# greysun/GraphEmbeddings

Hardware: AMD Instinct MI355X
Metric: scored triples/sec/GPU (d=200) (higher is better)
Workload: dtype f32

## Files before the change

### graphembeddings_amd/csrc/ge_launch.h

```cpp
#pragma once
#include <assert.h>
#include <hip/hip_runtime.h>
#include <stddef.h>
#include <stdint.h>

#include "ge_step_id.h"
#include "ge_sweep_route.h"
#include "ge_trans.h"

namespace ge {

struct TileGeom;
struct ShardOut;

int complex_max_dim();
int complex_score_launch(const float* table, int64_t N, int32_t d, const int32_t* triples, int64_t B, float max_norm,
                         int apply_sigmoid, float* out, hipStream_t st, int spectral = 0, float label = 0.f, float l2 = 0.f,
                         const float* table_sumsq = nullptr, int64_t ld = 0);
int complex_hinge_loss_launch(const float* table, int64_t N, int32_t d, const int32_t* pos, const int32_t* neg, int64_t B,
                              float margin, float max_norm, float* loss, float* sig_out, hipStream_t st, int spectral = 0);
int complex_hinge_grad_launch(const float* rows, int64_t N, int32_t d, const int32_t* pos, const int32_t* neg, int64_t B,
                              float margin, float lr, float max_norm, float* loss, int32_t* grad_idx, float* grad_val,
                              hipStream_t st, hipEvent_t ev_start = nullptr, hipEvent_t ev_stop = nullptr,
                              const int32_t* slot_item = nullptr, float* table_rw = nullptr, int spectral = 0,
                              const int32_t* order = nullptr);
int complex_logloss_grad_launch(const float* rows, int64_t N, int32_t d, const int32_t* triples, const float* labels,
                                int64_t M, float lr, float max_norm, float l2, const float* table_sumsq, float* loss,
                                int32_t* grad_idx, float* grad_val, hipStream_t st, const int32_t* negs = nullptr,
                                int64_t B = 0, float row_scale = 1.f, float neg_lr_eff = 0.f, hipEvent_t ev_start = nullptr,
                                hipEvent_t ev_stop = nullptr);
int shard_hinge_grad_launch(float* shard, int32_t d, const float* staged, const int32_t* pos_src, const int32_t* neg_src,
                            const int32_t* slot_item, int32_t R, int64_t B, float margin, float lr, float max_norm,
                            float* loss, int32_t* grad_idx, float* grad_val, float* gsum, int spectral, hipStream_t st,
                            hipEvent_t ev_start, hipEvent_t ev_stop, const int32_t* order, const float* const* peers,
                            int n_peers);
int table_sumsq_launch(const float* table, int64_t n, float* out, hipStream_t st);
int table_scale_launch(float* table, int64_t n, float factor, hipStream_t st);

int hole_score_launch(const float* table, int64_t N, int32_t d, const int32_t* triples, int64_t B, float max_norm,
                      int apply_sigmoid, float* out, hipStream_t st);
int hole_hinge_loss_launch(const float* table, int64_t N, int32_t d, const int32_t* pos, const int32_t* neg, int64_t B,
                           float margin, float max_norm, float* loss, float* sig_out, hipStream_t st);
int hole_hinge_grad_launch(const float* rows, int64_t N, int32_t d, const int32_t* pos, const int32_t* neg, int64_t B,
                           float margin, float lr, float max_norm, float* loss, int32_t* grad_idx, float* grad_val,
                           hipStream_t st, hipEvent_t ev_start = nullptr, hipEvent_t ev_stop = nullptr);

int hole_spectral_launch(float* table, int64_t N, int32_t d, int inverse, hipStream_t st);

int scatter_add_rows_launch(float* table, int64_t N, int32_t d, const int32_t* idx, const float* val, int64_t R,
                            hipStream_t st, hipEvent_t ev_start = nullptr, hipEvent_t ev_stop = nullptr);
int gather_rows_launch(const float* table, int64_t N, int32_t d, const int32_t* idx, int64_t R, float* out, hipStream_t st);
int corrupt_batch_launch(const int32_t* pos, int64_t B, const TypeSampler& ts, uint64_t step, int32_t* neg, hipStream_t st);
struct SamplerArgs {
  const int32_t* triples; int64_t T; const int64_t* bh_key; const int32_t* bh_ent; const int64_t* bt_key;
  const int32_t* bt_ent; int64_t n_known; const uint32_t* tail_threshold; int32_t n_rel, n_ent;
};
int bernoulli_corrupt_launch(const int32_t* pos, int64_t B, const SamplerArgs& s, int32_t ent_lo, uint64_t seed,
                             uint64_t step, int32_t* neg, hipStream_t st);
int select_rows_launch(const int32_t* valid, int64_t V, int64_t B, uint64_t seed, uint64_t counter, int32_t* out,
                       hipStream_t st);
int mean_pocket_launch(const float* loss, int64_t B, float* mean_out, float* best, int32_t* flag, hipStream_t st);
int copy_if_launch(const float* src, float* dst, int64_t n, const int32_t* flag, hipStream_t st);

int complex_score_1vK_launch(const float* table, int64_t N, int32_t d, const int32_t* hr, int64_t B, const int32_t* cand,
                             int64_t K, float max_norm, int apply_sigmoid, int cand_is_head, float* out, hipStream_t st);

struct SweepArgs {
  const float* table; int64_t N; int32_t d; const int32_t* hr; int64_t B; const int32_t* true_id; const int32_t* cand;
  int64_t K; float max_norm; int cand_is_head; const int32_t* known_off; const uint16_t* known_rc; int32_t* raw_cnt;
  int32_t* skip_cnt; float* true_loss; float* scores_out; int spec, scores_only, sweep_flags;
};
inline int table_mod16(const SweepArgs& a) { return (int)(reinterpret_cast<uintptr_t>(a.table) % 16); }
struct TopkOut { int32_t k; int32_t* out_id; float* out_loss; void* workspace; size_t workspace_bytes; };
struct SetArgs {
  const int32_t* row_set; const uint32_t* mask; int32_t n_sets;
  int64_t mw;
};

int complex_rank_1vK_launch(const SweepArgs& a, const void* planes_ws, hipStream_t st);

int pipe_sweep_launch(int cw, const SweepArgs& a, hipStream_t st);

int rank_planes_launch(const float* table, int64_t N, int32_t d, const int32_t* cand, int64_t K, float max_norm, int spec,
                       void* planes_ws, hipStream_t st);
int f16_sweep_launch(const SweepArgs& a, const void* planes_ws, hipStream_t st);
int topk_f16_launch(const SweepArgs& a, const TopkOut& t, const void* planes_ws, hipStream_t st);

int64_t candidate_mask_words(int64_t K);
int mask_from_classes_launch(const int32_t* cand_class, int64_t K, const uint32_t* allow, int32_t n_sets, int32_t n_class,
                             uint32_t* mask, hipStream_t st);
int mask_from_cells_launch(const int32_t* cells, int64_t M, int32_t n_sets, int64_t K, uint32_t* mask, hipStream_t st);
int masked_rank_launch(const SweepArgs& a, const SetArgs& sets, const void* planes_ws, hipStream_t st);
int masked_topk_launch(const SweepArgs& a, const TopkOut& t, const SetArgs& sets, const void* planes_ws, hipStream_t st);

int neighbor_max_k();
int neighbor_max_dim();
int64_t neighbor_planes_bytes(int64_t K, int32_t d);
int neighbor_planes_launch(const float* table, int64_t N, int32_t d, const int32_t* cand, int64_t K, void* planes_ws,
                           hipStream_t st);
size_t neighbor_ws_bytes(int64_t B, int64_t K, int32_t k);
int neighbor_dists_launch(const float* table, int64_t N, int32_t d, const int32_t* queries, int64_t B,
                          const int32_t* cand, int64_t K, int metric, const void* planes_ws, float* out, hipStream_t st);
int neighbor_topk_launch(const float* table, int64_t N, int32_t d, const int32_t* queries, int64_t B,
                         const int32_t* cand, int64_t K, int32_t k, int metric, int exclude_self, const void* planes_ws,
                         int32_t* out_id, float* out_dist, void* workspace, size_t workspace_bytes, hipStream_t st);

int known_cells_launch(int pass, const int64_t* key, const int64_t* ent, int64_t M, const int64_t* fixed, const int64_t* rel,
                       int64_t B, const int64_t* pos_of, int64_t n_rows, int64_t n_cand, int32_t* tile_cnt, int32_t* off,
                       uint16_t* rc, hipStream_t st);

size_t sort_scratch_bytes(int64_t n, int64_t n_sub, int64_t P);
unsigned long long* sort_scratch_keys(void* scratch);
int sort_tiles_launch(void* scratch, int64_t n, int64_t n_sub, int64_t P, int64_t n_rows, hipStream_t st,
                      const unsigned* limit, const unsigned long long** sorted);
int items_launch(const unsigned long long* sorted, int64_t n, const TileGeom& G, int direct, int32_t* out, const ShardOut* so,
                 hipStream_t st);
int relation_order_launch(const int32_t* triples, int64_t T, int64_t first_row, int64_t B, int64_t s0, int64_t n, int64_t N,
                          int32_t* out, int64_t stride, int64_t off_order, void* scratch, hipStream_t st);
size_t prep_big_scratch_bytes(int64_t B, int64_t negs, int64_t n);
int prepare_big_launch(const StepSeq& q, int64_t s0, int64_t n, const TypeSampler& ts, int direct, int32_t* out,
                       void* scratch, hipStream_t st, int negs);

int apply_items_launch(float* table, int d, const TileGeom& G, const int32_t* step_rec, const int32_t* gidx,
                       const float* gval, int split, float* out2, hipStream_t st, hipEvent_t ev_start, hipEvent_t ev_stop,
                       int det);
template <class T>
inline T* ws_at(void* base, size_t off) { return reinterpret_cast<T*>(reinterpret_cast<uintptr_t>(base) + off); }
struct HingeWs { int32_t* gidx; float* gval; size_t bytes; };
HingeWs hinge_ws(void* base, int64_t B, int32_t d);
struct LoglossWs { float* sumsq; int32_t* gidx; float* gval; size_t bytes; };
LoglossWs logloss_ws(void* base, int64_t M, int32_t d);
struct StepHyper {
  float lr0, decay_steps, decay_rate, max_norm;
  float lr_at(uint64_t gs) const { return decay_steps > 0.f ? lr0 / (1.0f + decay_rate * ((float)gs / decay_steps)) : lr0; }
};
size_t train_ws_bytes(int64_t B, int32_t d);
int train_steps_run(float* table, int32_t d, const StepSeq& q, int64_t n_steps, const TypeSampler& ts, float margin,
                    const StepHyper& hp, int model, float* loss, int keep_all_losses, int32_t* neg_ws, void* workspace,
                    size_t workspace_bytes, void** ev_pairs, int ev_kernel, void* pipe_handle, hipStream_t st);
size_t train_logloss_ws_bytes(int64_t B, int32_t negs, int32_t d);
int train_logloss_run(float* table, int32_t d, const StepSeq& q, int64_t n_steps, const TypeSampler& ts, int32_t negs,
                      float l2, const StepHyper& hp, float* loss, int keep_all_losses, int32_t* neg_ws, void* workspace,
                      size_t workspace_bytes, void* pipe_handle, hipStream_t st);
size_t train_prepare_bytes(int64_t B, int64_t n_steps);
int train_prepare_run(const StepSeq& q, int64_t n_steps, const TypeSampler& ts, int direct, int32_t* out, hipStream_t st);
void train_prepared_layout(int64_t B, int64_t* out);
int train_adagrad_run(float* table, float* accum, int32_t d, const StepSeq& q, int64_t n_steps, const TypeSampler& ts,
                      float margin, const StepHyper& hp, int model, float* loss, int keep_all_losses, int32_t* neg_ws,
                      void* workspace, size_t workspace_bytes, void* pipe_handle, hipStream_t st);
int pipeline_create(void** out);
int pipeline_reset(void* h);
int pipeline_destroy(void* h);

int adagrad_items_launch(float* table, float* accum, int d, const TileGeom& G, const int32_t* step_rec, const int32_t* gidx,
                         float* gval, float lr, hipStream_t st);
int adagrad_rows_launch(float* table, float* accum, int64_t N, int32_t d, const int32_t* idx, const float* val,
                        const int32_t* perm, int64_t R, float lr, hipStream_t st);

size_t shard_plan_scratch_bytes(int64_t B, int64_t S);
int shard_plan_launch(const int32_t* pos, const int32_t* neg, int64_t S, int64_t B, int64_t N, int32_t G, int32_t rank,
                      int32_t* records, int32_t* pos_src, int32_t* neg_src, int32_t* req_row, int32_t* counts,
                      void* scratch, int peer, hipStream_t st);
int shard_grad_launch(float* shard, int32_t d, const float* staged, const int32_t* pos_src, const int32_t* neg_src,
                      const int32_t* record, int32_t R, int64_t B, float margin, float lr, float max_norm, int spectral,
                      float* loss, int32_t* gidx, float* gval, float* gsum, const float* const* peers, int n_peers,
                      hipStream_t st, hipEvent_t e0, hipEvent_t e1);
int shard_apply_launch(float* shard, int32_t d, const int32_t* record, int64_t B, const int32_t* gidx, const float* gval,
                       int32_t R, float* gsum, hipStream_t st, hipEvent_t e0, hipEvent_t e1);
int64_t shard_owner_record_words(int64_t cap);
size_t shard_owner_scratch_bytes(int64_t cap, int64_t S);
int shard_owner_plan_launch(const int32_t* req_all, const int64_t* req_start, int64_t S, int64_t cap, int32_t rows_local,
                            int32_t* records, void* scratch, hipStream_t st);
int shard_owner_apply_launch(float* shard, int32_t d, const int32_t* record, int64_t cap, const float* recv, hipStream_t st);

int transx_max_dim();
size_t transx_ws_bytes(int64_t E, int64_t R, int32_t d, int64_t B);
int transx_score_launch(const TransModel& m, const int32_t* tri, int64_t B, float* out, hipStream_t st);
int transx_hinge_step_run(int model, int l1, float* ent, int64_t E, float* rel, int64_t R, float* normal,
                          float* ent_transfer, float* rel_transfer, int32_t d, const int32_t* pos, const int32_t* neg,
                          int64_t B, float margin, float lr, float* loss, void* workspace, size_t workspace_bytes,
                          hipStream_t st);
int transx_draw_launch(const SamplerArgs& s, int64_t B, uint64_t seed, uint64_t step, int32_t* pos, int32_t* neg,
                       hipStream_t st);
template <class Step>
int draw_then_step(const SamplerArgs& sa, int64_t B, uint64_t seed, uint64_t first_step, int64_t n_steps, int32_t* pos,
                   int32_t* neg, hipStream_t st, Step step) {
  for (int64_t s = 0; s < n_steps; ++s) {
    int rc = transx_draw_launch(sa, B, seed, first_step + (uint64_t)s, pos, neg, st);
    if (rc || (rc = step(s))) return rc;
  }
  return 0;
}
int transx_train_steps_run(int model, int l1, float* ent, int64_t E, float* rel, int64_t R, float* normal,
                           float* ent_transfer, float* rel_transfer, int32_t d, const SamplerArgs& sa, uint64_t seed,
                           uint64_t first_step, int64_t n_steps, int64_t B, float margin, float lr, float* losses,
                           void* workspace, size_t workspace_bytes, hipStream_t st);

int transr_max_dim();
size_t transr_ws_bytes(int64_t E, int64_t R, int32_t dE, int32_t dR, int64_t B);
int transr_score_launch(const TransModel& m, const int32_t* tri, int64_t B, float* out, hipStream_t st);
int transr_adam_step_run(int l1, float* ent, int64_t E, float* rel, float* rel_matrix, int64_t R, int32_t dE,
                         int32_t dR, float* m, float* v, const int32_t* pos, const int32_t* neg, int64_t B,
                         float margin, float lr, float b1, float b2, float eps, int64_t t, float* loss,
                         void* workspace, size_t workspace_bytes, hipStream_t st);
int transr_train_steps_run(int l1, float* ent, int64_t E, float* rel, float* rel_matrix, int64_t R, int32_t dE,
                           int32_t dR, float* m, float* v, const SamplerArgs& sa, uint64_t seed, uint64_t first_step,
                           int64_t n_steps, int64_t B, float margin, float lr, float b1, float b2, float eps,
                           int64_t first_t, float* losses, void* workspace, size_t workspace_bytes, hipStream_t st);

struct RankOut {
  const int32_t* known_off; const uint16_t* known_rc; int32_t* n_before; int32_t* n_known_before; float* true_dist;
  float* scores_out;
};

size_t trans_rank_ws_bytes(const TransModel& m, int64_t B);
int trans_rank_launch(const TransModel& m, const int32_t* tri, int64_t B, int cand_is_head, const RankOut& o,
                      void* workspace, size_t workspace_bytes, hipStream_t st);
int transx_topk_max_k();
size_t trans_topk_ws_bytes(const TransModel& m, int64_t B, int32_t k);
int trans_topk_launch(const TransModel& m, const int32_t* queries, int64_t B, int cand_is_head,
                      const int32_t* known_off, const uint16_t* known_rc, int32_t k, int32_t* out_id, float* out_dist,
                      void* workspace, size_t workspace_bytes, hipStream_t st);
int trans_rank_masked_launch(const TransModel& m, const int32_t* tri, int64_t B, int cand_is_head, const RankOut& o,
                             const SetArgs& sets, void* workspace, size_t workspace_bytes, hipStream_t st);
int trans_topk_masked_launch(const TransModel& m, const int32_t* queries, int64_t B, int cand_is_head,
                             const int32_t* known_off, const uint16_t* known_rc, int32_t k, int32_t* out_id,
                             float* out_dist, const SetArgs& sets, void* workspace, size_t workspace_bytes,
                             hipStream_t st);

size_t trans_relrank_ws_bytes(const TransModel& m, int64_t B);
int trans_relrank_launch(const TransModel& m, const int32_t* tri, int64_t B, const RankOut& o, void* workspace,
                         size_t workspace_bytes, hipStream_t st);

size_t threshold_fit_ws_bytes(int64_t M, int32_t n_seg);
int threshold_fit_launch(const float* score, const int32_t* seg, const uint8_t* label, int64_t M, int32_t n_seg,
                         float* thr_lo, float* thr_hi, int32_t* best_correct, int32_t* n_pos, int32_t* n_neg,
                         void* workspace, hipStream_t st);
int threshold_classify_launch(const float* score, const int32_t* seg, const uint8_t* label, int64_t M, int32_t n_seg,
                              const float* thr, uint8_t* pred, int32_t* confusion, hipStream_t st);

}
```

### graphembeddings_amd/csrc/ge_prep_big.hip

```cpp
#include "ge_prep.h"
#include "ge_launch.h"
#include <algorithm>

namespace ge {

__global__ __launch_bounds__(kPrepThreads) void prep_big_keys_kernel(
    const int32_t* __restrict__ triples, int64_t T, int64_t first_row, int64_t B, int64_t s0,
    const int32_t* __restrict__ id_to_type, int64_t N, const int64_t* __restrict__ type_offsets,
    int32_t n_types, const int32_t* __restrict__ type_ids, uint64_t seed, uint64_t global_step0,
    int32_t padded_size, int32_t mode, int direct, int negs, int32_t* __restrict__ prep,
    unsigned long long* __restrict__ keys_out) {
  const PrepLayout L = prep_layout(B, negs);
  const int tid = threadIdx.x, sub = blockIdx.y;
  const int64_t s = s0 + blockIdx.x;
  int32_t* rec = prep + (int64_t)blockIdx.x * L.stride;
  int32_t* slot_item = rec + L.off_slot;
  const int64_t i0 = (int64_t)sub * kSub;
  const int S = (int)((L.units - i0) < kSub ? (L.units - i0) : kSub);
  StepSource src{triples + 3 * step_row(first_row, T, B, s), B, id_to_type, N, type_offsets, n_types, type_ids, seed,
                 global_step0 + (uint64_t)s, padded_size, mode, negs};
  const bool batch_heads = (mode == GE_CORRUPT_BATCH_COIN) ? batch_coin_heads(seed, src.step) : false;
  unsigned long long* out = keys_out + ((int64_t)blockIdx.x * L.n_sub + sub) * L.P;
  if (direct)
    for (int i = tid; i < 6 * S; i += kPrepThreads) slot_item[6 * i0 + i] = -1;
  for (int il = tid; il < (int)L.S; il += kPrepThreads) {
    unsigned long long k[4] = {kInvalidKey, kInvalidKey, kInvalidKey, kInvalidKey};
    if (il < S) unit_keys(src, i0 + il, batch_heads, rec, k);
#pragma unroll
    for (int X = 0; X < 4; ++X)
      if (X < L.epu) out[L.epu * il + X] = k[X];
  }
}

__device__ __forceinline__ bool pass_is_identity(const unsigned* limit, int shift) {
  return limit && ((unsigned long long)(*limit) >> (shift - 32)) == 0ull;
}

__global__ __launch_bounds__(kPrepThreads) void prep_big_hist_kernel(
    const unsigned long long* __restrict__ src, int P, int n_sub, int shift, int bits, unsigned* __restrict__ hist,
    const unsigned* __restrict__ limit) {
  __shared__ unsigned cnt[kMaxRadix];
  if (pass_is_identity(limit, shift)) return;
  const int tid = threadIdx.x, tile = blockIdx.y;
  const int radix = 1 << bits;
  const unsigned dmask = (unsigned)radix - 1u;
  if (tid < radix) cnt[tid] = 0;
  __syncthreads();
  const unsigned long long* k = src + ((int64_t)blockIdx.x * n_sub + tile) * P;
  for (int i = tid; i < P; i += kPrepThreads) atomicAdd(&cnt[(unsigned)(k[i] >> shift) & dmask], 1u);
  __syncthreads();
  if (tid < radix) hist[((int64_t)blockIdx.x * radix + tid) * n_sub + tile] = cnt[tid];
}

__global__ __launch_bounds__(kPrepThreads) void prep_big_scatter_kernel(
    const unsigned long long* __restrict__ src, unsigned long long* __restrict__ dst,
    const unsigned* __restrict__ hist, int P, int n_sub, int shift, int bits, const unsigned* __restrict__ limit) {
  __shared__ unsigned whist[kMaxRadix * kPrepWaves];
  __shared__ unsigned gbase[kMaxRadix];
  __shared__ unsigned dstart[kMaxRadix];
  __shared__ unsigned wsum[4], wsum2[4];
  extern __shared__ __attribute__((aligned(16))) unsigned long long lkeys[];
  const int tid = threadIdx.x, lane = tid & (kWave - 1), wave = tid >> 6, tile = blockIdx.y;
  if (pass_is_identity(limit, shift)) {
    const int64_t o = ((int64_t)blockIdx.x * n_sub + tile) * P;
    for (int i = tid; i < P; i += kPrepThreads) dst[o + i] = src[o + i];
    return;
  }
  const int radix = 1 << bits, R = P / kPrepThreads, seg = kWave * R;
  const unsigned dmask = (unsigned)radix - 1u;
  const unsigned* h = hist + (int64_t)blockIdx.x * radix * n_sub;
  unsigned tot = 0, before = 0, mine = 0;
  if (tid < radix)
    for (int q = 0; q < n_sub; ++q) { const unsigned v = h[tid * n_sub + q]; if (q < tile) before += v; if (q == tile) mine = v; tot += v; }
  int incl = 0, incl2 = 0;
  if (tid < kMaxRadix) {
    incl = wave_incl_add((int)tot, lane);
    incl2 = wave_incl_add((int)mine, lane);
    if (lane == kWave - 1) { wsum[wave] = (unsigned)incl; wsum2[wave] = (unsigned)incl2; }
  }
  for (int i = tid; i < radix * kPrepWaves; i += kPrepThreads) whist[i] = 0;
  __syncthreads();
  if (tid < radix) {
    unsigned run = (unsigned)incl - tot, run2 = (unsigned)incl2 - mine;
    for (int w = 0; w < wave; ++w) { run += wsum[w]; run2 += wsum2[w]; }
    gbase[tid] = run + before;
    dstart[tid] = run2;
  }
  const unsigned long long* kin = src + ((int64_t)blockIdx.x * n_sub + tile) * P;
  unsigned long long k[16];
  unsigned off[16];
#pragma unroll
  for (int r = 0; r < 16; ++r)
    if (r < R) k[r] = kin[wave * seg + r * kWave + lane];
#pragma unroll
  for (int r = 0; r < 16; ++r) {
    if (r < R) {
      const unsigned dg = (unsigned)(k[r] >> shift) & dmask;
      unsigned long long peers = ~0ull;
      for (int b = 0; b < bits; ++b) {
        const bool bit = (dg >> b) & 1u;
        const unsigned long long bal = __ballot(bit);
        peers &= bit ? bal : ~bal;
      }
      const unsigned rank = (unsigned)__popcll(peers & ((1ull << lane) - 1ull));
      const unsigned cnt = (unsigned)__popcll(peers);
      unsigned* hp = whist + dg * kPrepWaves + wave;
      const unsigned base = *hp;
      __builtin_amdgcn_wave_barrier();
      if (rank == 0) *hp = base + cnt;
      __builtin_amdgcn_wave_barrier();
      off[r] = base + rank;
    }
  }
  __syncthreads();
  if (tid < radix) {
    unsigned run = 0;
    for (int w = 0; w < kPrepWaves; ++w) { const unsigned c = whist[tid * kPrepWaves + w]; whist[tid * kPrepWaves + w] = run; run += c; }
  }
  __syncthreads();
#pragma unroll
  for (int r = 0; r < 16; ++r) {
    if (r < R) {
      const unsigned dg = (unsigned)(k[r] >> shift) & dmask;
      lkeys[dstart[dg] + whist[dg * kPrepWaves + wave] + off[r]] = k[r];
    }
  }
  __syncthreads();
  unsigned long long* out = dst + (int64_t)blockIdx.x * n_sub * P;
  for (int i = tid; i < P; i += kPrepThreads) {
    const unsigned long long kk = lkeys[i];
    const unsigned dg = (unsigned)(kk >> shift) & dmask;
    out[gbase[dg] + ((unsigned)i - dstart[dg])] = kk;
  }
}

template <bool SHARD>
__global__ __launch_bounds__(kPrepThreads) void prep_big_items_kernel(
    const unsigned long long* __restrict__ sorted, TileGeom G, int direct, int32_t* __restrict__ prep, ShardOut so) {
  extern __shared__ __attribute__((aligned(16))) unsigned long long keys[];
  const int P = G.P, R = P / kPrepThreads, seg = kWave * R, n_sub = G.n_sub;
  int* wtot = reinterpret_cast<int*>(keys + P);
  const int tid = threadIdx.x, lane = tid & (kWave - 1), wave = tid >> 6, tile = blockIdx.y;
  const unsigned long long* g = sorted + (int64_t)blockIdx.x * n_sub * P;
  const int total = n_sub * P, base = tile * P;
  int32_t* rec = prep + (int64_t)blockIdx.x * G.stride;
  int32_t* slot_item = G.off_slot >= 0 ? rec + G.off_slot : nullptr;
  int32_t* subrec = rec + G.off_sub + tile * G.sub_stride;
  int32_t* items = subrec + G.off_items;
  int32_t* islots = subrec + G.off_islots;
  for (int i = tid; i < P; i += kPrepThreads) keys[i] = g[base + i];
  if (tid == 0) {
    int rs = -1;
    if (tile > 0) {
      const unsigned long long k0 = g[base], kp = g[base - 1];
      const uint32_t r0 = (uint32_t)(k0 >> 32);
      if (k0 != kInvalidKey && (uint32_t)(kp >> 32) == r0) {
        int lo = 0, hi = base - 1;
        while (lo < hi) { const int mid = (lo + hi) >> 1; if ((uint32_t)(g[mid] >> 32) < r0) lo = mid + 1; else hi = mid; }
        rs = lo;
      }
    }
    wtot[31] = rs;
    int before = 0;
    if (SHARD)
      for (int t = 0; t < tile; ++t) before += so.tile_heads[(int64_t)blockIdx.x * n_sub + t];
    wtot[30] = before;
  }
  __syncthreads();
  const int rs_in = wtot[31], u_before = wtot[30];
  auto key_at = [&](int i) -> unsigned long long {
    if (i >= 0 && i < P) return keys[i];
    const int gi = base + i;
    return (gi >= 0 && gi < total) ? g[gi] : kInvalidKey;
  };
  {
    int carry = -1;
    for (int r = 0; r < R; ++r) {
      const int i = wave * seg + r * kWave + lane;
      const unsigned long long kk = keys[i], kp = key_at(i - 1);
      const bool head = kk != kInvalidKey && (base + i == 0 || (uint32_t)(kp >> 32) != (uint32_t)(kk >> 32));
      const int m = max(wave_incl_max(head ? base + i : -1, lane), carry);
      carry = __shfl(m, kWave - 1, kWave);
    }
    if (lane == 0) wtot[wave] = carry;
  }
  __syncthreads();
  int prev_max = rs_in;
  for (int w = 0; w < wave; ++w) prev_max = max(prev_max, wtot[w]);
  __syncthreads();
  unsigned start_mask = 0, sole_mask = 0, rhead_mask = 0;
  int inc_loc[16], rs_loc[16];
  {
    int carry = 0, mcarry = prev_max;
#pragma unroll
    for (int r = 0; r < 16; ++r) {
      if (r < R) {
        const int i = wave * seg + r * kWave + lane;
        const unsigned long long kk = keys[i], kp = key_at(i - 1), kn = key_at(i + 1);
        const bool valid = kk != kInvalidKey;
        const uint32_t row = (uint32_t)(kk >> 32);
        const bool head = valid && (base + i == 0 || (uint32_t)(kp >> 32) != row);
        const bool sole = direct && head && !(kn != kInvalidKey && (uint32_t)(kn >> 32) == row) &&
                          !(SHARD && so.peer && row < (uint32_t)so.R);
        const bool rhead = SHARD && head && row >= (uint32_t)so.R;
        const int rs = max(wave_incl_max(head ? base + i : -1, lane), mcarry);
        mcarry = __shfl(rs, kWave - 1, kWave);
        rs_loc[r] = rs;
        const bool start = valid && ((base + i - rs) % kItemCap) == 0 && !sole;
        if (start) start_mask |= 1u << r;
        if (sole) sole_mask |= 1u << r;
        if (rhead) rhead_mask |= 1u << r;
        const int incl = wave_incl_add((start ? 1 : 0) | (rhead ? 1 << 16 : 0), lane) + carry;
        inc_loc[r] = incl;
        carry = __shfl(incl, kWave - 1, kWave);
      }
    }
    if (lane == 0) wtot[wave] = carry;
  }
  __syncthreads();
  int prev = 0, all = 0;
  for (int w = 0; w < kPrepWaves; ++w) { if (w < wave) prev += wtot[w]; all += wtot[w]; }
  if (tid == 0) subrec[0] = all & 0xFFFF;
  const int prev_items = prev & 0xFFFF, u0 = u_before + (prev >> 16) - 1;
#pragma unroll
  for (int r = 0; r < 16; ++r) {
    if (r < R) {
      const int i = wave * seg + r * kWave + lane;
      const unsigned long long kk = keys[i];
      const bool valid = kk != kInvalidKey;
      uint32_t row = (uint32_t)(kk >> 32);
      const uint32_t slot = (uint32_t)kk;
      const bool sole = (sole_mask >> r) & 1u;
      int tag = kSlotDirect;
      if (SHARD && valid) {
        const bool remote = row >= (uint32_t)so.R;
        const int u = u0 + (inc_loc[r] >> 16);
        uint32_t src = row;
        if (remote) {
          if ((rhead_mask >> r) & 1u) so.req_row[(int64_t)blockIdx.x * total + u] = (int32_t)(row % (uint32_t)so.R);
          if (!so.peer) src = (uint32_t)so.R + (uint32_t)u;
          row = (uint32_t)so.R + (uint32_t)u;
          tag = -3 - u;
        }
        const uint32_t pair = slot / 6u, X = slot - pair * 6u;
        if (X < 3) so.pos_src[((int64_t)blockIdx.x * so.B + pair) * 3 + X] = (int32_t)src;
        else so.neg_src[(int64_t)blockIdx.x * so.B + pair] = (int32_t)((src << 1) | (X - 3u));
      }
      if (sole) slot_item[slot] = tag;
      const bool is_start = (start_mask >> r) & 1u;
      unsigned long long sm = __ballot(is_start);
      const int idx_me = prev_items + (inc_loc[r] & 0xFFFF) - 1;
      const int g16 = lane >> 4, j16 = lane & 15;
      while (sm) {
        int srcl = -1;
#pragma unroll
        for (int g = 0; g < 4; ++g) {
          const int bpos = sm ? __builtin_ctzll(sm) : -1;
          if (sm) sm &= sm - 1;
          if (g == g16) srcl = bpos;
        }
        const int sl = srcl < 0 ? 0 : srcl;
        const int i_s = wave * seg + r * kWave + sl;
        const int idx_s = __shfl(idx_me, sl, kWave);
        const int row_s = __shfl((int)row, sl, kWave);
        const int rs_s = __shfl(rs_loc[r], sl, kWave);
        const unsigned long long k0 = key_at(i_s);
        const uint32_t krow = (uint32_t)(k0 >> 32);
        const unsigned long long kj = key_at(i_s + j16);
        const bool same = srcl >= 0 && kj != kInvalidKey && (uint32_t)(kj >> 32) == krow;
        const unsigned m16 = (unsigned)((__ballot(same) >> (16 * g16)) & 0xFFFFull);
        const int cnt = m16 == 0xFFFFu ? kItemCap : __builtin_ctz(~m16);
        if (srcl >= 0) {
          islots[idx_s * kItemCap + j16] = j16 < cnt ? (int32_t)(uint32_t)kj : -1;
          if (j16 == 0) {
            bool more = false;
            if (cnt == kItemCap) { const unsigned long long ke = key_at(i_s + kItemCap); more = ke != kInvalidKey && (uint32_t)(ke >> 32) == krow; }
            const bool multi = (base + i_s != rs_s) || more;
            items[2 * idx_s] = row_s;
            items[2 * idx_s + 1] = cnt | (multi ? (1 << 30) : 0);
          }
        }
      }
    }
  }
}

constexpr int kOrderP = 16384;
__global__ __launch_bounds__(kPrepThreads) void order_keys_kernel(
    const int32_t* __restrict__ triples, int64_t T, int64_t first_row, int64_t B, int64_t s0, int64_t N, int n_o,
    unsigned long long* __restrict__ keys_out, unsigned* __restrict__ limit) {
  const int64_t s = blockIdx.x;
  unsigned rmax = 0;
  const int32_t* pos = T > 0 ? triples + 3 * step_row(first_row, T, B, s0 + s) : triples + s * 3 * B;
  unsigned long long* out = keys_out + (s * n_o + blockIdx.y) * kOrderP;
  for (int i = threadIdx.x; i < kOrderP; i += kPrepThreads) {
    const int64_t j = (int64_t)blockIdx.y * kOrderP + i;
    unsigned long long k = kInvalidKey;
    if (j < B) {
      int32_t r = pos[3 * j + 2];
      if (r < 0 || r >= N) r = (int32_t)N;
      k = ((unsigned long long)(uint32_t)r << 32) | (uint32_t)j;
      rmax = max(rmax, (unsigned)r);
    }
    out[i] = k;
  }
#pragma unroll
  for (int m = 32; m >= 1; m >>= 1) rmax = max(rmax, (unsigned)__shfl_xor((int)rmax, m, kWave));
  if ((threadIdx.x & (kWave - 1)) == 0) atomicMax(limit, rmax);
}

__global__ __launch_bounds__(kPrepThreads) void order_write_kernel(
    const unsigned long long* __restrict__ sorted, int n_o, int64_t B, int64_t stride, int64_t off_order,
    int32_t* __restrict__ prep) {
  const unsigned long long* g = sorted + (int64_t)blockIdx.x * n_o * kOrderP;
  int32_t* order = prep + (int64_t)blockIdx.x * stride + off_order;
  for (int64_t i = (int64_t)blockIdx.y * kPrepThreads + threadIdx.x; i < B; i += (int64_t)gridDim.y * kPrepThreads)
    order[i] = (int32_t)(uint32_t)g[i];
}

size_t sort_scratch_bytes(int64_t n, int64_t n_sub, int64_t P) {
  const size_t keys = align_up(sizeof(unsigned long long) * (size_t)n * (size_t)n_sub * (size_t)P, 256);
  const size_t hist = align_up(sizeof(unsigned) * (size_t)n * kMaxRadix * (size_t)n_sub, 256);
  return 2 * keys + hist + 256;
}
static unsigned* sort_scratch_limit(void* scratch, int64_t n, int64_t n_sub, int64_t P) {
  return reinterpret_cast<unsigned*>(reinterpret_cast<char*>(scratch) + sort_scratch_bytes(n, n_sub, P) - 256);
}
unsigned long long* sort_scratch_keys(void* scratch) { return reinterpret_cast<unsigned long long*>(scratch); }

int sort_tiles_launch(void* scratch, int64_t n, int64_t n_sub, int64_t P, int64_t n_rows, hipStream_t st,
                      const unsigned* limit, const unsigned long long** sorted) {
  const SortBits sb = sort_bits_for(n_rows);
  const size_t keys_bytes = align_up(sizeof(unsigned long long) * (size_t)n * (size_t)n_sub * (size_t)P, 256);
  unsigned long long* ka = reinterpret_cast<unsigned long long*>(scratch);
  unsigned long long* kb = reinterpret_cast<unsigned long long*>(reinterpret_cast<char*>(scratch) + keys_bytes);
  unsigned* hist = reinterpret_cast<unsigned*>(reinterpret_cast<char*>(scratch) + 2 * keys_bytes);
  const dim3 grid((unsigned)n, (unsigned)n_sub), block(kPrepThreads);
  const size_t lds = sizeof(unsigned long long) * (size_t)P;
  const hipError_t e = hipFuncSetAttribute(reinterpret_cast<const void*>(prep_big_scatter_kernel),
                                           hipFuncAttributeMaxDynamicSharedMemorySize, 140 * 1024);
  if (e != hipSuccess) return (int)e;
  for (int pass = 0; pass < sb.n_pass; ++pass) {
    const int shift = 32 + pass * sb.bits;
    hipLaunchKernelGGL(prep_big_hist_kernel, grid, block, 0, st, ka, (int)P, (int)n_sub, shift, sb.bits, hist, limit);
    hipLaunchKernelGGL(prep_big_scatter_kernel, grid, block, lds, st, ka, kb, hist, (int)P, (int)n_sub, shift, sb.bits, limit);
    unsigned long long* t = ka; ka = kb; kb = t;
  }
  *sorted = ka;
  return launch_status();
}

int items_launch(const unsigned long long* sorted, int64_t n, const TileGeom& G, int direct, int32_t* out, const ShardOut* so,
                 hipStream_t st) {
  const size_t lds = sizeof(unsigned long long) * (size_t)G.P + sizeof(int) * 32;
  const dim3 grid((unsigned)n, (unsigned)G.n_sub), block(kPrepThreads);
  if (so) {
    hipError_t e = hipFuncSetAttribute(reinterpret_cast<const void*>(prep_big_items_kernel<true>),
                                       hipFuncAttributeMaxDynamicSharedMemorySize, 160 * 1024);
    if (e != hipSuccess) return (int)e;
    hipLaunchKernelGGL(prep_big_items_kernel<true>, grid, block, lds, st, sorted, G, direct, out, *so);
  } else {
    hipError_t e = hipFuncSetAttribute(reinterpret_cast<const void*>(prep_big_items_kernel<false>),
                                       hipFuncAttributeMaxDynamicSharedMemorySize, 160 * 1024);
    if (e != hipSuccess) return (int)e;
    hipLaunchKernelGGL(prep_big_items_kernel<false>, grid, block, lds, st, sorted, G, direct, out, ShardOut{});
  }
  return launch_status();
}

int relation_order_launch(const int32_t* triples, int64_t T, int64_t first_row, int64_t B, int64_t s0, int64_t n, int64_t N,
                          int32_t* out, int64_t stride, int64_t off_order, void* scratch, hipStream_t st) {
  const int n_o = (int)((B + kOrderP - 1) / kOrderP);
  unsigned* limit = sort_scratch_limit(scratch, n, n_o, kOrderP);
  if (hipMemsetAsync(limit, 0, sizeof(unsigned), st) != hipSuccess) return launch_status();
  hipLaunchKernelGGL(order_keys_kernel, dim3((unsigned)n, (unsigned)n_o), dim3(kPrepThreads), 0, st, triples, T, first_row, B,
                     s0, N, n_o, sort_scratch_keys(scratch), limit);
  const unsigned long long* sorted;
  const int rc = sort_tiles_launch(scratch, n, n_o, kOrderP, N + 1, st, limit, &sorted);
  if (rc) return rc;
  const int gy = (int)std::min<int64_t>((B + kPrepThreads - 1) / kPrepThreads, 64);
  hipLaunchKernelGGL(order_write_kernel, dim3((unsigned)n, (unsigned)gy), dim3(kPrepThreads), 0, st, sorted, n_o, B, stride,
                     off_order, out);
  return launch_status();
}

size_t prep_big_scratch_bytes(int64_t B, int64_t negs, int64_t n) {
  const PrepLayout L = prep_layout(B, negs);
  return L.n_sub <= 1 ? 0 : sort_scratch_bytes(n, L.n_sub, L.P);
}

int prepare_big_launch(const StepSeq& q, int64_t s0, int64_t n, const TypeSampler& ts, int direct, int32_t* out,
                       void* scratch, hipStream_t st, int negs) {
  const PrepLayout L = prep_layout(q.B, negs);
  const dim3 grid((unsigned)n, (unsigned)L.n_sub), block(kPrepThreads);
  hipLaunchKernelGGL(prep_big_keys_kernel, grid, block, 0, st, q.triples, q.T, q.first_row, q.B, s0, ts.id_to_type, ts.N,
                     ts.type_offsets, ts.n_types, ts.type_ids, ts.seed, q.global_step0, ts.padded_size, ts.mode, direct, negs,
                     out, sort_scratch_keys(scratch));
  const unsigned long long* sorted;
  int rc = sort_tiles_launch(scratch, n, L.n_sub, L.P, ts.N, st, nullptr, &sorted);
  if (rc) return rc;
  rc = items_launch(sorted, n, geom_of(L), direct, out, nullptr, st);
  if (rc || L.off_order < 0) return rc;
  return relation_order_launch(q.triples, q.T, q.first_row, q.B, s0, n, ts.N, out, L.stride, L.off_order, scratch, st);
}

}
```

### graphembeddings_amd/csrc/ge_shard.hip

```cpp
#include "ge_prep.h"
#include "ge_launch.h"

namespace ge {

__global__ __launch_bounds__(kPrepThreads) void shard_keys_kernel(
    const int32_t* __restrict__ pos, const int32_t* __restrict__ neg, int64_t B, int64_t N, int32_t G, int32_t rank,
    int32_t R, PrepLayout L, int32_t* __restrict__ prep, int32_t* __restrict__ pos_src, int32_t* __restrict__ neg_src,
    unsigned long long* __restrict__ keys_out) {
  const int tid = threadIdx.x, sub = blockIdx.y;
  const int64_t s = blockIdx.x;
  int32_t* slot_item = prep + s * L.stride + L.off_slot;
  const int64_t i0 = (int64_t)sub * kSub;
  const int S = (int)((B - i0) < kSub ? (B - i0) : kSub);
  unsigned long long* out = keys_out + (s * L.n_sub + sub) * L.P;
  for (int i = tid; i < 6 * S; i += kPrepThreads) slot_item[6 * i0 + i] = -1;
  auto vrow = [&](int32_t id) -> unsigned long long {
    const int32_t o = id % G, l = id / G;
    return (unsigned long long)(uint32_t)(o == rank ? l : R * (1 + o) + l);
  };
  for (int il = tid; il < (int)L.S; il += kPrepThreads) {
    unsigned long long k[4] = {kInvalidKey, kInvalidKey, kInvalidKey, kInvalidKey};
    if (il < S) {
      const int64_t i = i0 + il;
      const int32_t* p = pos + (s * B + i) * 3;
      const int32_t* n = neg + (s * B + i) * 3;
      const int32_t p0 = p[0], p1 = p[1], p2 = p[2], n0 = n[0], n1 = n[1], n2 = n[2];
      bool bad = p0 < 0 || p1 < 0 || p2 < 0 || p0 >= N || p1 >= N || p2 >= N || n0 < 0 || n1 < 0 || n0 >= N || n1 >= N;
      bad = bad || n2 != p2 || (n0 != p0 && n1 != p1);
      pos_src[(s * B + i) * 3] = -1; pos_src[(s * B + i) * 3 + 1] = -1; pos_src[(s * B + i) * 3 + 2] = -1;
      neg_src[s * B + i] = -1;
      if (!bad) {
        k[0] = (vrow(p0) << 32) | (uint32_t)(6 * i);
        k[1] = (vrow(p1) << 32) | (uint32_t)(6 * i + 1);
        k[2] = (vrow(p2) << 32) | (uint32_t)(6 * i + 2);
        if (n0 != p0) k[3] = (vrow(n0) << 32) | (uint32_t)(6 * i + 3);
        else if (n1 != p1) k[3] = (vrow(n1) << 32) | (uint32_t)(6 * i + 4);
      }
    }
#pragma unroll
    for (int X = 0; X < 4; ++X) out[4 * il + X] = k[X];
  }
}

__global__ __launch_bounds__(kPrepThreads) void shard_heads_kernel(
    const unsigned long long* __restrict__ sorted, int P, int n_sub, int32_t R, int32_t G, int32_t rank,
    int32_t* __restrict__ tile_heads, int32_t* __restrict__ counts) {
  __shared__ int own[64 + 1];
  const int tid = threadIdx.x, tile = blockIdx.y;
  const unsigned long long* g = sorted + (int64_t)blockIdx.x * n_sub * P;
  const int base = tile * P;
  if (tid <= 64) own[tid] = 0;
  __syncthreads();
  for (int i = tid; i < P; i += kPrepThreads) {
    const unsigned long long kk = g[base + i];
    if (kk == kInvalidKey) continue;
    const uint32_t row = (uint32_t)(kk >> 32);
    const bool head = (base + i == 0) || (uint32_t)(g[base + i - 1] >> 32) != row;
    if (!head) continue;
    if (row < (uint32_t)R) { atomicAdd(&own[rank], 1); continue; }
    atomicAdd(&own[row / (uint32_t)R - 1], 1);
    atomicAdd(&own[64], 1);
  }
  __syncthreads();
  if (tid < G && own[tid]) atomicAdd(&counts[(int64_t)blockIdx.x * G + tid], own[tid]);
  if (tid == 0) tile_heads[(int64_t)blockIdx.x * n_sub + tile] = own[64];
}

__global__ __launch_bounds__(kPrepThreads) void owner_keys_kernel(
    const int32_t* __restrict__ req_all, const int64_t* __restrict__ req_start, int P, int n_sub, int32_t rows_local,
    unsigned long long* __restrict__ keys_out) {
  const int64_t s = blockIdx.x;
  const int64_t b = req_start[s], n = req_start[s + 1] - b;
  unsigned long long* out = keys_out + (s * n_sub + blockIdx.y) * P;
  for (int i = threadIdx.x; i < P; i += kPrepThreads) {
    const int64_t j = (int64_t)blockIdx.y * P + i;
    unsigned long long k = kInvalidKey;
    if (j < n) {
      const int32_t row = req_all[b + j];
      if (row >= 0 && row < rows_local) k = ((unsigned long long)(uint32_t)row << 32) | (uint32_t)j;
    }
    out[i] = k;
  }
}

size_t shard_plan_scratch_bytes(int64_t B, int64_t S) {
  const PrepLayout L = prep_layout(B);
  return sort_scratch_bytes(S, L.n_sub, L.P) + align_up(sizeof(int32_t) * (size_t)S * (size_t)L.n_sub, 256);
}

int shard_plan_launch(const int32_t* pos, const int32_t* neg, int64_t S, int64_t B, int64_t N, int32_t G, int32_t rank,
                      int32_t* records, int32_t* pos_src, int32_t* neg_src, int32_t* req_row, int32_t* counts,
                      void* scratch, int peer, hipStream_t st) {
  const PrepLayout L = prep_layout(B);
  const int32_t R = (int32_t)((N + G - 1) / G);
  const dim3 grid((unsigned)S, (unsigned)L.n_sub), block(kPrepThreads);
  int32_t* tile_heads = reinterpret_cast<int32_t*>(reinterpret_cast<char*>(scratch) + sort_scratch_bytes(S, L.n_sub, L.P));
  hipError_t e = hipMemsetAsync(counts, 0, sizeof(int32_t) * (size_t)S * (size_t)G, st);
  if (e != hipSuccess) return (int)e;
  hipLaunchKernelGGL(shard_keys_kernel, grid, block, 0, st, pos, neg, B, N, G, rank, R, L, records, pos_src, neg_src,
                     sort_scratch_keys(scratch));
  const unsigned long long* sorted;
  int rc = sort_tiles_launch(scratch, S, L.n_sub, L.P, (int64_t)R * (G + 1), st, nullptr, &sorted);
  if (rc) return rc;
  hipLaunchKernelGGL(shard_heads_kernel, grid, block, 0, st, sorted, (int)L.P, (int)L.n_sub, R, G, rank, tile_heads, counts);
  const ShardOut so{R, B, pos_src, neg_src, req_row, tile_heads, peer ? 1 : 0};
  rc = items_launch(sorted, S, geom_of(L), 1, records, &so, st);
  if (rc || L.off_order < 0) return rc;
  return relation_order_launch(pos, 0, 0, B, 0, S, N, records, L.stride, L.off_order, scratch, st);
}

int shard_grad_launch(float* shard, int32_t d, const float* staged, const int32_t* pos_src, const int32_t* neg_src,
                      const int32_t* record, int32_t R, int64_t B, float margin, float lr, float max_norm, int spectral,
                      float* loss, int32_t* gidx, float* gval, float* gsum, const float* const* peers, int n_peers,
                      hipStream_t st, hipEvent_t e0, hipEvent_t e1) {
  const PrepLayout L = prep_layout(B);
  return shard_hinge_grad_launch(shard, d, staged, pos_src, neg_src, record + L.off_slot, R, B, margin, lr, max_norm, loss,
                                 gidx, gval, gsum, spectral, st, e0, e1, L.off_order >= 0 ? record + L.off_order : nullptr,
                                 peers, n_peers);
}

int shard_apply_launch(float* shard, int32_t d, const int32_t* record, int64_t B, const int32_t* gidx, const float* gval,
                       int32_t R, float* gsum, hipStream_t st, hipEvent_t e0, hipEvent_t e1) {
  return apply_items_launch(shard, d, geom_of(prep_layout(B)), record, gidx, gval, R, gsum, st, e0, e1, 0);
}

constexpr int kOwnerP = 16384;
static inline int owner_tiles(int64_t cap) { return (int)((cap + kOwnerP - 1) / kOwnerP); }
int64_t shard_owner_record_words(int64_t cap) { return cap <= 0 ? 0 : geom_plain(kOwnerP, owner_tiles(cap)).stride; }
size_t shard_owner_scratch_bytes(int64_t cap, int64_t S) { return cap <= 0 ? 0 : sort_scratch_bytes(S, owner_tiles(cap), kOwnerP); }

int shard_owner_plan_launch(const int32_t* req_all, const int64_t* req_start, int64_t S, int64_t cap, int32_t rows_local,
                            int32_t* records, void* scratch, hipStream_t st) {
  if (cap <= 0 || S <= 0) return 0;
  const int n_sub = owner_tiles(cap);
  const dim3 grid((unsigned)S, (unsigned)n_sub), block(kPrepThreads);
  hipLaunchKernelGGL(owner_keys_kernel, grid, block, 0, st, req_all, req_start, kOwnerP, n_sub, rows_local,
                     sort_scratch_keys(scratch));
  const unsigned long long* sorted;
  const int rc = sort_tiles_launch(scratch, S, n_sub, kOwnerP, rows_local, st, nullptr, &sorted);
  if (rc) return rc;
  return items_launch(sorted, S, geom_plain(kOwnerP, n_sub), 0, records, nullptr, st);
}

int shard_owner_apply_launch(float* shard, int32_t d, const int32_t* record, int64_t cap, const float* recv, hipStream_t st) {
  if (cap <= 0) return 0;
  return apply_items_launch(shard, d, geom_plain(kOwnerP, owner_tiles(cap)), record, nullptr, recv, 0x7FFFFFFF, nullptr, st,
                            nullptr, nullptr, 0);
}

}
```

Baseline: 593.9 million.

## Restructure prep radix sort into fixed-span blocks with fused key counting

Reworks the per-step radix sort used in batch preparation. Tiles of up to P keys per block become fixed 4096-key spans of 256-thread blocks processed in 1024-key rounds with static shared memory. The key-generation kernel now also builds the first-pass histogram, so one count kernel is skipped. The items kernel is split into a counting launch and a writing launch over 1024-key spans. The aim is more blocks, higher occupancy and no large dynamic LDS, at the cost of extra launches, more histogram traffic and more complex carry logic across spans.

```diff
diff --git a/graphembeddings_amd/csrc/ge_launch.h b/graphembeddings_amd/csrc/ge_launch.h
--- a/graphembeddings_amd/csrc/ge_launch.h
+++ b/graphembeddings_amd/csrc/ge_launch.h
@@ -112,9 +112,9 @@
 size_t sort_scratch_bytes(int64_t n, int64_t n_sub, int64_t P);
 unsigned long long* sort_scratch_keys(void* scratch);
 int sort_tiles_launch(void* scratch, int64_t n, int64_t n_sub, int64_t P, int64_t n_rows, hipStream_t st,
-                      const unsigned* limit, const unsigned long long** sorted);
+                      const unsigned long long** sorted);
 int items_launch(const unsigned long long* sorted, int64_t n, const TileGeom& G, int direct, int32_t* out, const ShardOut* so,
-                 hipStream_t st);
+                 void* scratch, hipStream_t st);
 int relation_order_launch(const int32_t* triples, int64_t T, int64_t first_row, int64_t B, int64_t s0, int64_t n, int64_t N,
                           int32_t* out, int64_t stride, int64_t off_order, void* scratch, hipStream_t st);
 size_t prep_big_scratch_bytes(int64_t B, int64_t negs, int64_t n);
diff --git a/graphembeddings_amd/csrc/ge_prep_big.hip b/graphembeddings_amd/csrc/ge_prep_big.hip
--- a/graphembeddings_amd/csrc/ge_prep_big.hip
+++ b/graphembeddings_amd/csrc/ge_prep_big.hip
@@ -4,97 +4,132 @@
 
 namespace ge {
 
-__global__ __launch_bounds__(kPrepThreads) void prep_big_keys_kernel(
+constexpr int kBigThreads = 256;
+constexpr int kBigWaves = kBigThreads / kWave;
+constexpr int kSortRound = 1024;
+constexpr int kSortR = kSortRound / kBigThreads;
+constexpr int kSortSpan = 4096;
+constexpr int kItemSpan = 1024;
+constexpr int kItemR = kItemSpan / kBigThreads;
+constexpr int kKeyUnits = 1024;
+static_assert(kMaxRadix <= kBigThreads, "one digit per thread in the scans");
+static_assert(kSortSpan % kSortRound == 0 && kSortRound % kBigThreads == 0 && kItemSpan % kBigThreads == 0, "geometry");
+
+static inline int64_t sort_spans(int64_t total) { return (total + kSortSpan - 1) / kSortSpan; }
+
+__device__ __forceinline__ void count_write(const unsigned* lcnt, unsigned* __restrict__ cnt, int n_span, int radix) {
+  if ((int)threadIdx.x < radix) cnt[((int64_t)blockIdx.x * n_span + blockIdx.y) * radix + threadIdx.x] = lcnt[threadIdx.x];
+}
+
+__global__ __launch_bounds__(kBigThreads) void prep_big_keys_kernel(
     const int32_t* __restrict__ triples, int64_t T, int64_t first_row, int64_t B, int64_t s0,
     const int32_t* __restrict__ id_to_type, int64_t N, const int64_t* __restrict__ type_offsets,
     int32_t n_types, const int32_t* __restrict__ type_ids, uint64_t seed, uint64_t global_step0,
     int32_t padded_size, int32_t mode, int direct, int negs, int32_t* __restrict__ prep,
-    unsigned long long* __restrict__ keys_out) {
+    unsigned long long* __restrict__ keys_out, unsigned* __restrict__ cnt, int bits) {
+  __shared__ unsigned lcnt[kMaxRadix];
   const PrepLayout L = prep_layout(B, negs);
-  const int tid = threadIdx.x, sub = blockIdx.y;
+  const int tid = threadIdx.x;
   const int64_t s = s0 + blockIdx.x;
   int32_t* rec = prep + (int64_t)blockIdx.x * L.stride;
   int32_t* slot_item = rec + L.off_slot;
-  const int64_t i0 = (int64_t)sub * kSub;
-  const int S = (int)((L.units - i0) < kSub ? (L.units - i0) : kSub);
+  const int pu0 = blockIdx.y * kKeyUnits, pu_end = (int)(L.n_sub * L.S), S = (int)L.S, units = (int)L.units;
   StepSource src{triples + 3 * step_row(first_row, T, B, s), B, id_to_type, N, type_offsets, n_types, type_ids, seed,
                  global_step0 + (uint64_t)s, padded_size, mode, negs};
   const bool batch_heads = (mode == GE_CORRUPT_BATCH_COIN) ? batch_coin_heads(seed, src.step) : false;
-  unsigned long long* out = keys_out + ((int64_t)blockIdx.x * L.n_sub + sub) * L.P;
+  unsigned long long* out = keys_out + (int64_t)blockIdx.x * L.n_sub * L.P;
+  const unsigned dmask = (1u << bits) - 1u;
+  if (cnt) {
+    lcnt[tid] = 0;
+    __syncthreads();
+  }
   if (direct)
-    for (int i = tid; i < 6 * S; i += kPrepThreads) slot_item[6 * i0 + i] = -1;
-  for (int il = tid; il < (int)L.S; il += kPrepThreads) {
+    for (int i = tid; i < 6 * kKeyUnits; i += kBigThreads) {
+      const int pu = pu0 + i / 6, tile = pu / S, j = tile * (int)kSub + (pu - tile * S);
+      if (pu < pu_end && j < units) slot_item[6 * (int64_t)j + i % 6] = -1;
+    }
+  for (int u = tid; u < kKeyUnits; u += kBigThreads) {
+    const int pu = pu0 + u;
+    if (pu >= pu_end) break;
+    const int tile = pu / S, j = tile * (int)kSub + (pu - tile * S);
     unsigned long long k[4] = {kInvalidKey, kInvalidKey, kInvalidKey, kInvalidKey};
-    if (il < S) unit_keys(src, i0 + il, batch_heads, rec, k);
+    if (j < units) unit_keys(src, j, batch_heads, rec, k);
 #pragma unroll
     for (int X = 0; X < 4; ++X)
-      if (X < L.epu) out[L.epu * il + X] = k[X];
+      if (X < L.epu) {
+        out[L.epu * (int64_t)pu + X] = k[X];
+        if (cnt) atomicAdd(&lcnt[(unsigned)(k[X] >> 32) & dmask], 1u);
+      }
+  }
+  if (cnt) {
+    __syncthreads();
+    count_write(lcnt, cnt, (int)gridDim.y, 1 << bits);
   }
 }
 
 __device__ __forceinline__ bool pass_is_identity(const unsigned* limit, int shift) {
   return limit && ((unsigned long long)(*limit) >> (shift - 32)) == 0ull;
 }
-
-__global__ __launch_bounds__(kPrepThreads) void prep_big_hist_kernel(
-    const unsigned long long* __restrict__ src, int P, int n_sub, int shift, int bits, unsigned* __restrict__ hist,
+__device__ __forceinline__ const unsigned long long* sorted_of(const unsigned long long* ka, const unsigned long long* kb,
+                                                               const unsigned* limit, int n_pass, int bits) {
+  int m = 0;
+  for (int p = 0; p < n_pass; ++p) m += pass_is_identity(limit, 32 + p * bits) ? 0 : 1;
+  return (m & 1) ? kb : ka;
+}
+
+__global__ __launch_bounds__(kBigThreads) void sort_count_kernel(
+    const unsigned long long* __restrict__ src, int total, int shift, int bits, unsigned* __restrict__ cnt,
     const unsigned* __restrict__ limit) {
-  __shared__ unsigned cnt[kMaxRadix];
+  __shared__ unsigned lcnt[kMaxRadix];
   if (pass_is_identity(limit, shift)) return;
-  const int tid = threadIdx.x, tile = blockIdx.y;
+  const int tid = threadIdx.x;
+  const unsigned dmask = (1u << bits) - 1u;
+  lcnt[tid] = 0;
+  __syncthreads();
+  const int p0 = blockIdx.y * kSortSpan, p1 = min(p0 + kSortSpan, total);
+  const unsigned long long* k = src + (int64_t)blockIdx.x * total;
+  for (int i = p0 + tid; i < p1; i += kBigThreads) atomicAdd(&lcnt[(unsigned)(k[i] >> shift) & dmask], 1u);
+  __syncthreads();
+  count_write(lcnt, cnt, (int)gridDim.y, 1 << bits);
+}
+
+__global__ __launch_bounds__(kBigThreads) void sort_scatter_kernel(
+    const unsigned long long* __restrict__ src, unsigned long long* __restrict__ dst, const unsigned* __restrict__ cnt,
+    int total, int shift, int bits, const unsigned* __restrict__ limit) {
+  __shared__ __attribute__((aligned(16))) unsigned long long lkeys[kSortRound];
+  __shared__ unsigned whist[kBigWaves * kMaxRadix];
+  __shared__ unsigned gbase[kMaxRadix];
+  __shared__ unsigned dstart[kMaxRadix];
+  __shared__ unsigned wsum[kBigWaves], wsum2[kBigWaves];
+  if (pass_is_identity(limit, shift)) return;
+  const int tid = threadIdx.x, lane = tid & (kWave - 1), wave = tid >> 6, span = blockIdx.y, n_span = gridDim.y;
   const int radix = 1 << bits;
   const unsigned dmask = (unsigned)radix - 1u;
-  if (tid < radix) cnt[tid] = 0;
-  __syncthreads();
-  const unsigned long long* k = src + ((int64_t)blockIdx.x * n_sub + tile) * P;
-  for (int i = tid; i < P; i += kPrepThreads) atomicAdd(&cnt[(unsigned)(k[i] >> shift) & dmask], 1u);
-  __syncthreads();
-  if (tid < radix) hist[((int64_t)blockIdx.x * radix + tid) * n_sub + tile] = cnt[tid];
-}
-
-__global__ __launch_bounds__(kPrepThreads) void prep_big_scatter_kernel(
-    const unsigned long long* __restrict__ src, unsigned long long* __restrict__ dst,
-    const unsigned* __restrict__ hist, int P, int n_sub, int shift, int bits, const unsigned* __restrict__ limit) {
-  __shared__ unsigned whist[kMaxRadix * kPrepWaves];
-  __shared__ unsigned gbase[kMaxRadix];
-  __shared__ unsigned dstart[kMaxRadix];
-  __shared__ unsigned wsum[4], wsum2[4];
-  extern __shared__ __attribute__((aligned(16))) unsigned long long lkeys[];
-  const int tid = threadIdx.x, lane = tid & (kWave - 1), wave = tid >> 6, tile = blockIdx.y;
-  if (pass_is_identity(limit, shift)) {
-    const int64_t o = ((int64_t)blockIdx.x * n_sub + tile) * P;
-    for (int i = tid; i < P; i += kPrepThreads) dst[o + i] = src[o + i];
-    return;
-  }
-  const int radix = 1 << bits, R = P / kPrepThreads, seg = kWave * R;
-  const unsigned dmask = (unsigned)radix - 1u;
-  const unsigned* h = hist + (int64_t)blockIdx.x * radix * n_sub;
-  unsigned tot = 0, before = 0, mine = 0;
-  if (tid < radix)
-    for (int q = 0; q < n_sub; ++q) { const unsigned v = h[tid * n_sub + q]; if (q < tile) before += v; if (q == tile) mine = v; tot += v; }
-  int incl = 0, incl2 = 0;
-  if (tid < kMaxRadix) {
-    incl = wave_incl_add((int)tot, lane);
-    incl2 = wave_incl_add((int)mine, lane);
-    if (lane == kWave - 1) { wsum[wave] = (unsigned)incl; wsum2[wave] = (unsigned)incl2; }
-  }
-  for (int i = tid; i < radix * kPrepWaves; i += kPrepThreads) whist[i] = 0;
-  __syncthreads();
+  unsigned tot = 0, before = 0;
   if (tid < radix) {
-    unsigned run = (unsigned)incl - tot, run2 = (unsigned)incl2 - mine;
-    for (int w = 0; w < wave; ++w) { run += wsum[w]; run2 += wsum2[w]; }
-    gbase[tid] = run + before;
-    dstart[tid] = run2;
-  }
-  const unsigned long long* kin = src + ((int64_t)blockIdx.x * n_sub + tile) * P;
-  unsigned long long k[16];
-  unsigned off[16];
-#pragma unroll
-  for (int r = 0; r < 16; ++r)
-    if (r < R) k[r] = kin[wave * seg + r * kWave + lane];
-#pragma unroll
-  for (int r = 0; r < 16; ++r) {
-    if (r < R) {
+    const unsigned* h = cnt + (int64_t)blockIdx.x * n_span * radix + tid;
+#pragma unroll 4
+    for (int q = 0; q < n_span; ++q) { const unsigned v = h[(int64_t)q * radix]; if (q < span) before += v; tot += v; }
+  }
+  const int incl = wave_incl_add((int)tot, lane);
+  if (lane == kWave - 1) wsum[wave] = (unsigned)incl;
+  __syncthreads();
+  unsigned my_base = (unsigned)incl - tot + before;
+#pragma unroll
+  for (int w = 0; w < kBigWaves; ++w) my_base += w < wave ? wsum[w] : 0u;
+  gbase[tid] = my_base;
+  const int p0 = span * kSortSpan, rounds = min(kSortSpan, total - p0) / kSortRound;
+  const unsigned long long* kin = src + (int64_t)blockIdx.x * total + p0;
+  unsigned long long* out = dst + (int64_t)blockIdx.x * total;
+  for (int t = 0; t < rounds; ++t) {
+    for (int i = tid; i < kMaxRadix * kBigWaves; i += kBigThreads) whist[i] = 0;
+    __syncthreads();
+    unsigned long long k[kSortR];
+    unsigned off[kSortR];
+#pragma unroll
+    for (int r = 0; r < kSortR; ++r) k[r] = kin[t * kSortRound + wave * (kWave * kSortR) + r * kWave + lane];
+#pragma unroll
+    for (int r = 0; r < kSortR; ++r) {
       const unsigned dg = (unsigned)(k[r] >> shift) & dmask;
       unsigned long long peers = ~0ull;
       for (int b = 0; b < bits; ++b) {
@@ -103,55 +138,65 @@
         peers &= bit ? bal : ~bal;
       }
       const unsigned rank = (unsigned)__popcll(peers & ((1ull << lane) - 1ull));
-      const unsigned cnt = (unsigned)__popcll(peers);
-      unsigned* hp = whist + dg * kPrepWaves + wave;
+      const unsigned c = (unsigned)__popcll(peers);
+      unsigned* hp = whist + wave * kMaxRadix + dg;
       const unsigned base = *hp;
       __builtin_amdgcn_wave_barrier();
-      if (rank == 0) *hp = base + cnt;
+      if (rank == 0) *hp = base + c;
       __builtin_amdgcn_wave_barrier();
       off[r] = base + rank;
     }
-  }
-  __syncthreads();
-  if (tid < radix) {
-    unsigned run = 0;
-    for (int w = 0; w < kPrepWaves; ++w) { const unsigned c = whist[tid * kPrepWaves + w]; whist[tid * kPrepWaves + w] = run; run += c; }
-  }
-  __syncthreads();
-#pragma unroll
-  for (int r = 0; r < 16; ++r) {
-    if (r < R) {
+    __syncthreads();
+    unsigned mine = 0;
+    if (tid < radix)
+      for (int w = 0; w < kBigWaves; ++w) { const unsigned c = whist[w * kMaxRadix + tid]; whist[w * kMaxRadix + tid] = mine; mine += c; }
+    const int incl2 = wave_incl_add((int)mine, lane);
+    if (lane == kWave - 1) wsum2[wave] = (unsigned)incl2;
+    __syncthreads();
+    unsigned ds = (unsigned)incl2 - mine;
+#pragma unroll
+    for (int w = 0; w < kBigWaves; ++w) ds += w < wave ? wsum2[w] : 0u;
+    dstart[tid] = ds;
+    __syncthreads();
+#pragma unroll
+    for (int r = 0; r < kSortR; ++r) {
       const unsigned dg = (unsigned)(k[r] >> shift) & dmask;
-      lkeys[dstart[dg] + whist[dg * kPrepWaves + wave] + off[r]] = k[r];
-    }
-  }
-  __syncthreads();
-  unsigned long long* out = dst + (int64_t)blockIdx.x * n_sub * P;
-  for (int i = tid; i < P; i += kPrepThreads) {
-    const unsigned long long kk = lkeys[i];
-    const unsigned dg = (unsigned)(kk >> shift) & dmask;
-    out[gbase[dg] + ((unsigned)i - dstart[dg])] = kk;
-  }
-}
-
-template <bool SHARD>
-__global__ __launch_bounds__(kPrepThreads) void prep_big_items_kernel(
-    const unsigned long long* __restrict__ sorted, TileGeom G, int direct, int32_t* __restrict__ prep, ShardOut so) {
-  extern __shared__ __attribute__((aligned(16))) unsigned long long keys[];
-  const int P = G.P, R = P / kPrepThreads, seg = kWave * R, n_sub = G.n_sub;
-  int* wtot = reinterpret_cast<int*>(keys + P);
-  const int tid = threadIdx.x, lane = tid & (kWave - 1), wave = tid >> 6, tile = blockIdx.y;
+      lkeys[dstart[dg] + whist[wave * kMaxRadix + dg] + off[r]] = k[r];
+    }
+    __syncthreads();
+    for (int i = tid; i < kSortRound; i += kBigThreads) {
+      const unsigned long long kk = lkeys[i];
+      const unsigned dg = (unsigned)(kk >> shift) & dmask;
+      out[gbase[dg] + ((unsigned)i - dstart[dg])] = kk;
+    }
+    __syncthreads();
+    my_base += mine;
+    gbase[tid] = my_base;
+  }
+}
+
+template <bool SHARD, bool COUNT>
+__global__ __launch_bounds__(kBigThreads) void items_kernel(
+    const unsigned long long* __restrict__ sorted, TileGeom G, int direct, int32_t* __restrict__ prep, ShardOut so,
+    int32_t* __restrict__ span_cnt) {
+  __shared__ __attribute__((aligned(16))) unsigned long long keys[kItemSpan];
+  __shared__ int wtot[kBigWaves], carry_in[3];
+  constexpr int seg = kWave * kItemR;
+  const int P = G.P, n_sub = G.n_sub, spt = P / kItemSpan;
+  const int tid = threadIdx.x, lane = tid & (kWave - 1), wave = tid >> 6;
+  const int tile = blockIdx.y / spt, sp = blockIdx.y - tile * spt;
   const unsigned long long* g = sorted + (int64_t)blockIdx.x * n_sub * P;
-  const int total = n_sub * P, base = tile * P;
+  const int total = n_sub * P, base = blockIdx.y * kItemSpan;
+  int32_t* cnt_tile = span_cnt + ((int64_t)blockIdx.x * n_sub + tile) * spt;
   int32_t* rec = prep + (int64_t)blockIdx.x * G.stride;
   int32_t* slot_item = G.off_slot >= 0 ? rec + G.off_slot : nullptr;
   int32_t* subrec = rec + G.off_sub + tile * G.sub_stride;
   int32_t* items = subrec + G.off_items;
   int32_t* islots = subrec + G.off_islots;
-  for (int i = tid; i < P; i += kPrepThreads) keys[i] = g[base + i];
+  for (int i = tid; i < kItemSpan; i += kBigThreads) keys[i] = g[base + i];
   if (tid == 0) {
     int rs = -1;
-    if (tile > 0) {
+    if (base > 0) {
       const unsigned long long k0 = g[base], kp = g[base - 1];
       const uint32_t r0 = (uint32_t)(k0 >> 32);
       if (k0 != kInvalidKey && (uint32_t)(kp >> 32) == r0) {
@@ -160,22 +205,29 @@
         rs = lo;
       }
     }
-    wtot[31] = rs;
-    int before = 0;
-    if (SHARD)
-      for (int t = 0; t < tile; ++t) before += so.tile_heads[(int64_t)blockIdx.x * n_sub + t];
-    wtot[30] = before;
-  }
-  __syncthreads();
-  const int rs_in = wtot[31], u_before = wtot[30];
+    carry_in[0] = rs;
+    if (!COUNT) {
+      int prev = 0, all = 0;
+      for (int q = 0; q < spt; ++q) { const int c = cnt_tile[q]; if (q < sp) prev += c; all += c; }
+      int before = 0;
+      if (SHARD)
+        for (int t = 0; t < tile; ++t) before += so.tile_heads[(int64_t)blockIdx.x * n_sub + t];
+      carry_in[1] = prev;
+      carry_in[2] = before;
+      if (sp == 0) subrec[0] = all & 0xFFFF;
+    }
+  }
+  __syncthreads();
+  const int rs_in = carry_in[0];
   auto key_at = [&](int i) -> unsigned long long {
-    if (i >= 0 && i < P) return keys[i];
+    if (i >= 0 && i < kItemSpan) return keys[i];
     const int gi = base + i;
     return (gi >= 0 && gi < total) ? g[gi] : kInvalidKey;
   };
   {
     int carry = -1;
-    for (int r = 0; r < R; ++r) {
+#pragma unroll
+    for (int r = 0; r < kItemR; ++r) {
       const int i = wave * seg + r * kWave + lane;
       const unsigned long long kk = keys[i], kp = key_at(i - 1);
       const bool head = kk != kInvalidKey && (base + i == 0 || (uint32_t)(kp >> 32) != (uint32_t)(kk >> 32));
@@ -189,181 +241,189 @@
   for (int w = 0; w < wave; ++w) prev_max = max(prev_max, wtot[w]);
   __syncthreads();
   unsigned start_mask = 0, sole_mask = 0, rhead_mask = 0;
-  int inc_loc[16], rs_loc[16];
+  int inc_loc[kItemR], rs_loc[kItemR];
   {
     int carry = 0, mcarry = prev_max;
 #pragma unroll
-    for (int r = 0; r < 16; ++r) {
-      if (r < R) {
-        const int i = wave * seg + r * kWave + lane;
-        const unsigned long long kk = keys[i], kp = key_at(i - 1), kn = key_at(i + 1);
-        const bool valid = kk != kInvalidKey;
-        const uint32_t row = (uint32_t)(kk >> 32);
-        const bool head = valid && (base + i == 0 || (uint32_t)(kp >> 32) != row);
-        const bool sole = direct && head && !(kn != kInvalidKey && (uint32_t)(kn >> 32) == row) &&
-                          !(SHARD && so.peer && row < (uint32_t)so.R);
-        const bool rhead = SHARD && head && row >= (uint32_t)so.R;
-        const int rs = max(wave_incl_max(head ? base + i : -1, lane), mcarry);
-        mcarry = __shfl(rs, kWave - 1, kWave);
-        rs_loc[r] = rs;
-        const bool start = valid && ((base + i - rs) % kItemCap) == 0 && !sole;
-        if (start) start_mask |= 1u << r;
-        if (sole) sole_mask |= 1u << r;
-        if (rhead) rhead_mask |= 1u << r;
-        const int incl = wave_incl_add((start ? 1 : 0) | (rhead ? 1 << 16 : 0), lane) + carry;
-        inc_loc[r] = incl;
-        carry = __shfl(incl, kWave - 1, kWave);
-      }
+    for (int r = 0; r < kItemR; ++r) {
+      const int i = wave * seg + r * kWave + lane;
+      const unsigned long long kk = keys[i], kp = key_at(i - 1), kn = key_at(i + 1);
+      const bool valid = kk != kInvalidKey;
+      const uint32_t row = (uint32_t)(kk >> 32);
+      const bool head = valid && (base + i == 0 || (uint32_t)(kp >> 32) != row);
+      const bool sole = direct && head && !(kn != kInvalidKey && (uint32_t)(kn >> 32) == row) &&
+                        !(SHARD && so.peer && row < (uint32_t)so.R);
+      const bool rhead = SHARD && head && row >= (uint32_t)so.R;
+      const int rs = max(wave_incl_max(head ? base + i : -1, lane), mcarry);
+      mcarry = __shfl(rs, kWave - 1, kWave);
+      rs_loc[r] = rs;
+      const bool start = valid && ((base + i - rs) % kItemCap) == 0 && !sole;
+      if (start) start_mask |= 1u << r;
+      if (sole) sole_mask |= 1u << r;
+      if (rhead) rhead_mask |= 1u << r;
+      const int incl = wave_incl_add((start ? 1 : 0) | (rhead ? 1 << 16 : 0), lane) + carry;
+      inc_loc[r] = incl;
+      carry = __shfl(incl, kWave - 1, kWave);
     }
     if (lane == 0) wtot[wave] = carry;
   }
   __syncthreads();
-  int prev = 0, all = 0;
-  for (int w = 0; w < kPrepWaves; ++w) { if (w < wave) prev += wtot[w]; all += wtot[w]; }
-  if (tid == 0) subrec[0] = all & 0xFFFF;
-  const int prev_items = prev & 0xFFFF, u0 = u_before + (prev >> 16) - 1;
-#pragma unroll
-  for (int r = 0; r < 16; ++r) {
-    if (r < R) {
-      const int i = wave * seg + r * kWave + lane;
-      const unsigned long long kk = keys[i];
-      const bool valid = kk != kInvalidKey;
-      uint32_t row = (uint32_t)(kk >> 32);
-      const uint32_t slot = (uint32_t)kk;
-      const bool sole = (sole_mask >> r) & 1u;
-      int tag = kSlotDirect;
-      if (SHARD && valid) {
-        const bool remote = row >= (uint32_t)so.R;
-        const int u = u0 + (inc_loc[r] >> 16);
-        uint32_t src = row;
-        if (remote) {
-          if ((rhead_mask >> r) & 1u) so.req_row[(int64_t)blockIdx.x * total + u] = (int32_t)(row % (uint32_t)so.R);
-          if (!so.peer) src = (uint32_t)so.R + (uint32_t)u;
-          row = (uint32_t)so.R + (uint32_t)u;
-          tag = -3 - u;
+  if (COUNT) {
+    if (tid == 0) { int all = 0; for (int w = 0; w < kBigWaves; ++w) all += wtot[w]; cnt_tile[sp] = all; }
+    return;
+  }
+  int prev = carry_in[1];
+  for (int w = 0; w < wave; ++w) prev += wtot[w];
+  const int prev_items = prev & 0xFFFF, u0 = carry_in[2] + (prev >> 16) - 1;
+#pragma unroll
+  for (int r = 0; r < kItemR; ++r) {
+    const int i = wave * seg + r * kWave + lane;
+    const unsigned long long kk = keys[i];
+    const bool valid = kk != kInvalidKey;
+    uint32_t row = (uint32_t)(kk >> 32);
+    const uint32_t slot = (uint32_t)kk;
+    const bool sole = (sole_mask >> r) & 1u;
+    int tag = kSlotDirect;
+    if (SHARD && valid) {
+      const bool remote = row >= (uint32_t)so.R;
+      const int u = u0 + (inc_loc[r] >> 16);
+      uint32_t src = row;
+      if (remote) {
+        if ((rhead_mask >> r) & 1u) so.req_row[(int64_t)blockIdx.x * total + u] = (int32_t)(row % (uint32_t)so.R);
+        if (!so.peer) src = (uint32_t)so.R + (uint32_t)u;
+        row = (uint32_t)so.R + (uint32_t)u;
+        tag = -3 - u;
+      }
+      const uint32_t pair = slot / 6u, X = slot - pair * 6u;
+      if (X < 3) so.pos_src[((int64_t)blockIdx.x * so.B + pair) * 3 + X] = (int32_t)src;
+      else so.neg_src[(int64_t)blockIdx.x * so.B + pair] = (int32_t)((src << 1) | (X - 3u));
+    }
+    if (sole) slot_item[slot] = tag;
+    const bool is_start = (start_mask >> r) & 1u;
+    unsigned long long sm = __ballot(is_start);
+    const int idx_me = prev_items + (inc_loc[r] & 0xFFFF) - 1;
+    const int g16 = lane >> 4, j16 = lane & 15;
+    while (sm) {
+      int srcl = -1;
+#pragma unroll
+      for (int gq = 0; gq < 4; ++gq) {
+        const int bpos = sm ? __builtin_ctzll(sm) : -1;
+        if (sm) sm &= sm - 1;
+        if (gq == g16) srcl = bpos;
+      }
+      const int sl = srcl < 0 ? 0 : srcl;
+      const int i_s = wave * seg + r * kWave + sl;
+      const int idx_s = __shfl(idx_me, sl, kWave);
+      const int row_s = __shfl((int)row, sl, kWave);
+      const int rs_s = __shfl(rs_loc[r], sl, kWave);
+      const unsigned long long k0 = key_at(i_s);
+      const uint32_t krow = (uint32_t)(k0 >> 32);
+      const unsigned long long kj = key_at(i_s + j16);
+      const bool same = srcl >= 0 && kj != kInvalidKey && (uint32_t)(kj >> 32) == krow;
+      const unsigned m16 = (unsigned)((__ballot(same) >> (16 * g16)) & 0xFFFFull);
+      const int cnt = m16 == 0xFFFFu ? kItemCap : __builtin_ctz(~m16);
+      if (srcl >= 0) {
+        islots[idx_s * kItemCap + j16] = j16 < cnt ? (int32_t)(uint32_t)kj : -1;
+        if (j16 == 0) {
+          bool more = false;
+          if (cnt == kItemCap) { const unsigned long long ke = key_at(i_s + kItemCap); more = ke != kInvalidKey && (uint32_t)(ke >> 32) == krow; }
+          const bool multi = (base + i_s != rs_s) || more;
+          items[2 * idx_s] = row_s;
+          items[2 * idx_s + 1] = cnt | (multi ? (1 << 30) : 0);
         }
-        const uint32_t pair = slot / 6u, X = slot - pair * 6u;
-        if (X < 3) so.pos_src[((int64_t)blockIdx.x * so.B + pair) * 3 + X] = (int32_t)src;
-        else so.neg_src[(int64_t)blockIdx.x * so.B + pair] = (int32_t)((src << 1) | (X - 3u));
-      }
-      if (sole) slot_item[slot] = tag;
-      const bool is_start = (start_mask >> r) & 1u;
-      unsigned long long sm = __ballot(is_start);
-      const int idx_me = prev_items + (inc_loc[r] & 0xFFFF) - 1;
-      const int g16 = lane >> 4, j16 = lane & 15;
-      while (sm) {
-        int srcl = -1;
-#pragma unroll
-        for (int g = 0; g < 4; ++g) {
-          const int bpos = sm ? __builtin_ctzll(sm) : -1;
-          if (sm) sm &= sm - 1;
-          if (g == g16) srcl = bpos;
-        }
-        const int sl = srcl < 0 ? 0 : srcl;
-        const int i_s = wave * seg + r * kWave + sl;
-        const int idx_s = __shfl(idx_me, sl, kWave);
-        const int row_s = __shfl((int)row, sl, kWave);
-        const int rs_s = __shfl(rs_loc[r], sl, kWave);
-        const unsigned long long k0 = key_at(i_s);
-        const uint32_t krow = (uint32_t)(k0 >> 32);
-        const unsigned long long kj = key_at(i_s + j16);
-        const bool same = srcl >= 0 && kj != kInvalidKey && (uint32_t)(kj >> 32) == krow;
-        const unsigned m16 = (unsigned)((__ballot(same) >> (16 * g16)) & 0xFFFFull);
-        const int cnt = m16 == 0xFFFFu ? kItemCap : __builtin_ctz(~m16);
-        if (srcl >= 0) {
-          islots[idx_s * kItemCap + j16] = j16 < cnt ? (int32_t)(uint32_t)kj : -1;
-          if (j16 == 0) {
-            bool more = false;
-            if (cnt == kItemCap) { const unsigned long long ke = key_at(i_s + kItemCap); more = ke != kInvalidKey && (uint32_t)(ke >> 32) == krow; }
-            const bool multi = (base + i_s != rs_s) || more;
-            items[2 * idx_s] = row_s;
-            items[2 * idx_s + 1] = cnt | (multi ? (1 << 30) : 0);
-          }
-        }
       }
     }
   }
 }
 
 constexpr int kOrderP = 16384;
-__global__ __launch_bounds__(kPrepThreads) void order_keys_kernel(
-    const int32_t* __restrict__ triples, int64_t T, int64_t first_row, int64_t B, int64_t s0, int64_t N, int n_o,
-    unsigned long long* __restrict__ keys_out, unsigned* __restrict__ limit) {
+__global__ __launch_bounds__(kBigThreads) void order_keys_kernel(
+    const int32_t* __restrict__ triples, int64_t T, int64_t first_row, int64_t B, int64_t s0, int64_t N, int total,
+    unsigned long long* __restrict__ keys_out, unsigned* __restrict__ limit, unsigned* __restrict__ cnt, int bits) {
+  __shared__ unsigned lcnt[kMaxRadix];
   const int64_t s = blockIdx.x;
+  const unsigned dmask = (1u << bits) - 1u;
   unsigned rmax = 0;
   const int32_t* pos = T > 0 ? triples + 3 * step_row(first_row, T, B, s0 + s) : triples + s * 3 * B;
-  unsigned long long* out = keys_out + (s * n_o + blockIdx.y) * kOrderP;
-  for (int i = threadIdx.x; i < kOrderP; i += kPrepThreads) {
-    const int64_t j = (int64_t)blockIdx.y * kOrderP + i;
+  unsigned long long* out = keys_out + s * total;
+  lcnt[threadIdx.x] = 0;
+  __syncthreads();
+  const int p0 = blockIdx.y * kSortSpan, p1 = min(p0 + kSortSpan, total);
+  for (int j = p0 + threadIdx.x; j < p1; j += kBigThreads) {
     unsigned long long k = kInvalidKey;
     if (j < B) {
-      int32_t r = pos[3 * j + 2];
+      int32_t r = pos[3 * (int64_t)j + 2];
       if (r < 0 || r >= N) r = (int32_t)N;
       k = ((unsigned long long)(uint32_t)r << 32) | (uint32_t)j;
       rmax = max(rmax, (unsigned)r);
     }
-    out[i] = k;
+    out[j] = k;
+    atomicAdd(&lcnt[(unsigned)(k >> 32) & dmask], 1u);
   }
 #pragma unroll
   for (int m = 32; m >= 1; m >>= 1) rmax = max(rmax, (unsigned)__shfl_xor((int)rmax, m, kWave));
   if ((threadIdx.x & (kWave - 1)) == 0) atomicMax(limit, rmax);
-}
-
-__global__ __launch_bounds__(kPrepThreads) void order_write_kernel(
-    const unsigned long long* __restrict__ sorted, int n_o, int64_t B, int64_t stride, int64_t off_order,
-    int32_t* __restrict__ prep) {
-  const unsigned long long* g = sorted + (int64_t)blockIdx.x * n_o * kOrderP;
+  __syncthreads();
+  count_write(lcnt, cnt, (int)gridDim.y, 1 << bits);
+}
+
+__global__ __launch_bounds__(kBigThreads) void order_write_kernel(
+    const unsigned long long* __restrict__ ka, const unsigned long long* __restrict__ kb, const unsigned* __restrict__ limit,
+    int n_pass, int bits, int total, int64_t B, int64_t stride, int64_t off_order, int32_t* __restrict__ prep) {
+  const unsigned long long* g = sorted_of(ka, kb, limit, n_pass, bits) + (int64_t)blockIdx.x * total;
   int32_t* order = prep + (int64_t)blockIdx.x * stride + off_order;
-  for (int64_t i = (int64_t)blockIdx.y * kPrepThreads + threadIdx.x; i < B; i += (int64_t)gridDim.y * kPrepThreads)
+  for (int64_t i = (int64_t)blockIdx.y * kBigThreads + threadIdx.x; i < B; i += (int64_t)gridDim.y * kBigThreads)
     order[i] = (int32_t)(uint32_t)g[i];
 }
 
-size_t sort_scratch_bytes(int64_t n, int64_t n_sub, int64_t P) {
+struct SortScratch { unsigned long long *ka, *kb; unsigned *cnt, *limit; size_t bytes; };
+static SortScratch sort_scratch(void* scratch, int64_t n, int64_t n_sub, int64_t P) {
   const size_t keys = align_up(sizeof(unsigned long long) * (size_t)n * (size_t)n_sub * (size_t)P, 256);
-  const size_t hist = align_up(sizeof(unsigned) * (size_t)n * kMaxRadix * (size_t)n_sub, 256);
-  return 2 * keys + hist + 256;
-}
-static unsigned* sort_scratch_limit(void* scratch, int64_t n, int64_t n_sub, int64_t P) {
-  return reinterpret_cast<unsigned*>(reinterpret_cast<char*>(scratch) + sort_scratch_bytes(n, n_sub, P) - 256);
-}
+  const size_t cnt = align_up(sizeof(unsigned) * (size_t)n * kMaxRadix * (size_t)sort_spans(n_sub * P), 256);
+  return SortScratch{ws_at<unsigned long long>(scratch, 0), ws_at<unsigned long long>(scratch, keys),
+                     ws_at<unsigned>(scratch, 2 * keys), ws_at<unsigned>(scratch, 2 * keys + cnt), 2 * keys + cnt + 256};
+}
+size_t sort_scratch_bytes(int64_t n, int64_t n_sub, int64_t P) { return sort_scratch(nullptr, n, n_sub, P).bytes; }
 unsigned long long* sort_scratch_keys(void* scratch) { return reinterpret_cast<unsigned long long*>(scratch); }
 
-int sort_tiles_launch(void* scratch, int64_t n, int64_t n_sub, int64_t P, int64_t n_rows, hipStream_t st,
-                      const unsigned* limit, const unsigned long long** sorted) {
-  const SortBits sb = sort_bits_for(n_rows);
-  const size_t keys_bytes = align_up(sizeof(unsigned long long) * (size_t)n * (size_t)n_sub * (size_t)P, 256);
-  unsigned long long* ka = reinterpret_cast<unsigned long long*>(scratch);
-  unsigned long long* kb = reinterpret_cast<unsigned long long*>(reinterpret_cast<char*>(scratch) + keys_bytes);
-  unsigned* hist = reinterpret_cast<unsigned*>(reinterpret_cast<char*>(scratch) + 2 * keys_bytes);
-  const dim3 grid((unsigned)n, (unsigned)n_sub), block(kPrepThreads);
-  const size_t lds = sizeof(unsigned long long) * (size_t)P;
-  const hipError_t e = hipFuncSetAttribute(reinterpret_cast<const void*>(prep_big_scatter_kernel),
-                                           hipFuncAttributeMaxDynamicSharedMemorySize, 140 * 1024);
-  if (e != hipSuccess) return (int)e;
+static void sort_passes(const SortScratch& w, int64_t n, int64_t total, SortBits sb, bool counted0, const unsigned* limit,
+                        hipStream_t st) {
+  const dim3 grid((unsigned)n, (unsigned)sort_spans(total)), block(kBigThreads);
+  unsigned long long *ka = w.ka, *kb = w.kb;
   for (int pass = 0; pass < sb.n_pass; ++pass) {
     const int shift = 32 + pass * sb.bits;
-    hipLaunchKernelGGL(prep_big_hist_kernel, grid, block, 0, st, ka, (int)P, (int)n_sub, shift, sb.bits, hist, limit);
-    hipLaunchKernelGGL(prep_big_scatter_kernel, grid, block, lds, st, ka, kb, hist, (int)P, (int)n_sub, shift, sb.bits, limit);
-    unsigned long long* t = ka; ka = kb; kb = t;
-  }
-  *sorted = ka;
+    if (pass > 0 || !counted0)
+      hipLaunchKernelGGL(sort_count_kernel, grid, block, 0, st, ka, (int)total, shift, sb.bits, w.cnt, limit);
+    hipLaunchKernelGGL(sort_scatter_kernel, grid, block, 0, st, ka, kb, w.cnt, (int)total, shift, sb.bits, limit);
+#ifdef GE_EXP_PREP_REPEAT
+    for (int rep = 1; rep < GE_EXP_PREP_REPEAT; ++rep)
+      hipLaunchKernelGGL(sort_scatter_kernel, grid, block, 0, st, ka, kb, w.cnt, (int)total, shift, sb.bits, limit);
+#endif
+    std::swap(ka, kb);
+  }
+}
+
+int sort_tiles_launch(void* scratch, int64_t n, int64_t n_sub, int64_t P, int64_t n_rows, hipStream_t st,
+                      const unsigned long long** sorted) {
+  if (P % kSortRound) return GE_EINVAL;
+  const SortScratch w = sort_scratch(scratch, n, n_sub, P);
+  const SortBits sb = sort_bits_for(n_rows);
+  sort_passes(w, n, n_sub * P, sb, false, nullptr, st);
+  *sorted = (sb.n_pass & 1) ? w.kb : w.ka;
   return launch_status();
 }
 
 int items_launch(const unsigned long long* sorted, int64_t n, const TileGeom& G, int direct, int32_t* out, const ShardOut* so,
-                 hipStream_t st) {
-  const size_t lds = sizeof(unsigned long long) * (size_t)G.P + sizeof(int) * 32;
-  const dim3 grid((unsigned)n, (unsigned)G.n_sub), block(kPrepThreads);
+                 void* scratch, hipStream_t st) {
+  if (G.P % kItemSpan) return GE_EINVAL;
+  int32_t* span_cnt = reinterpret_cast<int32_t*>(sort_scratch(scratch, n, G.n_sub, G.P).cnt);
+  const dim3 grid((unsigned)n, (unsigned)(G.n_sub * (G.P / kItemSpan))), block(kBigThreads);
   if (so) {
-    hipError_t e = hipFuncSetAttribute(reinterpret_cast<const void*>(prep_big_items_kernel<true>),
-                                       hipFuncAttributeMaxDynamicSharedMemorySize, 160 * 1024);
-    if (e != hipSuccess) return (int)e;
-    hipLaunchKernelGGL(prep_big_items_kernel<true>, grid, block, lds, st, sorted, G, direct, out, *so);
+    hipLaunchKernelGGL((items_kernel<true, true>), grid, block, 0, st, sorted, G, direct, out, *so, span_cnt);
+    hipLaunchKernelGGL((items_kernel<true, false>), grid, block, 0, st, sorted, G, direct, out, *so, span_cnt);
   } else {
-    hipError_t e = hipFuncSetAttribute(reinterpret_cast<const void*>(prep_big_items_kernel<false>),
-                                       hipFuncAttributeMaxDynamicSharedMemorySize, 160 * 1024);
-    if (e != hipSuccess) return (int)e;
-    hipLaunchKernelGGL(prep_big_items_kernel<false>, grid, block, lds, st, sorted, G, direct, out, ShardOut{});
+    hipLaunchKernelGGL((items_kernel<false, true>), grid, block, 0, st, sorted, G, direct, out, ShardOut{}, span_cnt);
+    hipLaunchKernelGGL((items_kernel<false, false>), grid, block, 0, st, sorted, G, direct, out, ShardOut{}, span_cnt);
   }
   return launch_status();
 }
@@ -371,16 +431,16 @@
 int relation_order_launch(const int32_t* triples, int64_t T, int64_t first_row, int64_t B, int64_t s0, int64_t n, int64_t N,
                           int32_t* out, int64_t stride, int64_t off_order, void* scratch, hipStream_t st) {
   const int n_o = (int)((B + kOrderP - 1) / kOrderP);
-  unsigned* limit = sort_scratch_limit(scratch, n, n_o, kOrderP);
-  if (hipMemsetAsync(limit, 0, sizeof(unsigned), st) != hipSuccess) return launch_status();
-  hipLaunchKernelGGL(order_keys_kernel, dim3((unsigned)n, (unsigned)n_o), dim3(kPrepThreads), 0, st, triples, T, first_row, B,
-                     s0, N, n_o, sort_scratch_keys(scratch), limit);
-  const unsigned long long* sorted;
-  const int rc = sort_tiles_launch(scratch, n, n_o, kOrderP, N + 1, st, limit, &sorted);
-  if (rc) return rc;
-  const int gy = (int)std::min<int64_t>((B + kPrepThreads - 1) / kPrepThreads, 64);
-  hipLaunchKernelGGL(order_write_kernel, dim3((unsigned)n, (unsigned)gy), dim3(kPrepThreads), 0, st, sorted, n_o, B, stride,
-                     off_order, out);
+  const int64_t total = (int64_t)n_o * kOrderP;
+  const SortScratch w = sort_scratch(scratch, n, n_o, kOrderP);
+  const SortBits sb = sort_bits_for(N + 1);
+  if (hipMemsetAsync(w.limit, 0, sizeof(unsigned), st) != hipSuccess) return launch_status();
+  hipLaunchKernelGGL(order_keys_kernel, dim3((unsigned)n, (unsigned)sort_spans(total)), dim3(kBigThreads), 0, st, triples, T,
+                     first_row, B, s0, N, (int)total, w.ka, w.limit, w.cnt, sb.bits);
+  sort_passes(w, n, total, sb, true, w.limit, st);
+  const int gy = (int)std::min<int64_t>((B + kBigThreads - 1) / kBigThreads, 64);
+  hipLaunchKernelGGL(order_write_kernel, dim3((unsigned)n, (unsigned)gy), dim3(kBigThreads), 0, st, w.ka, w.kb, w.limit,
+                     sb.n_pass, sb.bits, (int)total, B, stride, off_order, out);
   return launch_status();
 }
 
@@ -392,14 +452,15 @@
 int prepare_big_launch(const StepSeq& q, int64_t s0, int64_t n, const TypeSampler& ts, int direct, int32_t* out,
                        void* scratch, hipStream_t st, int negs) {
   const PrepLayout L = prep_layout(q.B, negs);
-  const dim3 grid((unsigned)n, (unsigned)L.n_sub), block(kPrepThreads);
-  hipLaunchKernelGGL(prep_big_keys_kernel, grid, block, 0, st, q.triples, q.T, q.first_row, q.B, s0, ts.id_to_type, ts.N,
-                     ts.type_offsets, ts.n_types, ts.type_ids, ts.seed, q.global_step0, ts.padded_size, ts.mode, direct, negs,
-                     out, sort_scratch_keys(scratch));
-  const unsigned long long* sorted;
-  int rc = sort_tiles_launch(scratch, n, L.n_sub, L.P, ts.N, st, nullptr, &sorted);
-  if (rc) return rc;
-  rc = items_launch(sorted, n, geom_of(L), direct, out, nullptr, st);
+  const SortScratch w = sort_scratch(scratch, n, L.n_sub, L.P);
+  const SortBits sb = sort_bits_for(ts.N);
+  const int64_t total = L.n_sub * L.P, n_blk = (L.n_sub * L.S + kKeyUnits - 1) / kKeyUnits;
+  const bool counted0 = L.epu * kKeyUnits == kSortSpan;
+  hipLaunchKernelGGL(prep_big_keys_kernel, dim3((unsigned)n, (unsigned)n_blk), dim3(kBigThreads), 0, st, q.triples, q.T,
+                     q.first_row, q.B, s0, ts.id_to_type, ts.N, ts.type_offsets, ts.n_types, ts.type_ids, ts.seed,
+                     q.global_step0, ts.padded_size, ts.mode, direct, negs, out, w.ka, counted0 ? w.cnt : nullptr, sb.bits);
+  sort_passes(w, n, total, sb, counted0, nullptr, st);
+  int rc = items_launch((sb.n_pass & 1) ? w.kb : w.ka, n, geom_of(L), direct, out, nullptr, scratch, st);
   if (rc || L.off_order < 0) return rc;
   return relation_order_launch(q.triples, q.T, q.first_row, q.B, s0, n, ts.N, out, L.stride, L.off_order, scratch, st);
 }
diff --git a/graphembeddings_amd/csrc/ge_shard.hip b/graphembeddings_amd/csrc/ge_shard.hip
--- a/graphembeddings_amd/csrc/ge_shard.hip
+++ b/graphembeddings_amd/csrc/ge_shard.hip
@@ -100,11 +100,11 @@
   hipLaunchKernelGGL(shard_keys_kernel, grid, block, 0, st, pos, neg, B, N, G, rank, R, L, records, pos_src, neg_src,
                      sort_scratch_keys(scratch));
   const unsigned long long* sorted;
-  int rc = sort_tiles_launch(scratch, S, L.n_sub, L.P, (int64_t)R * (G + 1), st, nullptr, &sorted);
+  int rc = sort_tiles_launch(scratch, S, L.n_sub, L.P, (int64_t)R * (G + 1), st, &sorted);
   if (rc) return rc;
   hipLaunchKernelGGL(shard_heads_kernel, grid, block, 0, st, sorted, (int)L.P, (int)L.n_sub, R, G, rank, tile_heads, counts);
   const ShardOut so{R, B, pos_src, neg_src, req_row, tile_heads, peer ? 1 : 0};
-  rc = items_launch(sorted, S, geom_of(L), 1, records, &so, st);
+  rc = items_launch(sorted, S, geom_of(L), 1, records, &so, scratch, st);
   if (rc || L.off_order < 0) return rc;
   return relation_order_launch(pos, 0, 0, B, 0, S, N, records, L.stride, L.off_order, scratch, st);
 }
@@ -137,9 +137,9 @@
   hipLaunchKernelGGL(owner_keys_kernel, grid, block, 0, st, req_all, req_start, kOwnerP, n_sub, rows_local,
                      sort_scratch_keys(scratch));
   const unsigned long long* sorted;
-  const int rc = sort_tiles_launch(scratch, S, n_sub, kOwnerP, rows_local, st, nullptr, &sorted);
+  const int rc = sort_tiles_launch(scratch, S, n_sub, kOwnerP, rows_local, st, &sorted);
   if (rc) return rc;
-  return items_launch(sorted, S, geom_plain(kOwnerP, n_sub), 0, records, nullptr, st);
+  return items_launch(sorted, S, geom_plain(kOwnerP, n_sub), 0, records, nullptr, scratch, st);
 }
 
 int shard_owner_apply_launch(float* shard, int32_t d, const int32_t* record, int64_t cap, const float* recv, hipStream_t st) {
```

Result: no change. 593.6 million, median of 2 (-0.1%).
